# MinghanLi/UniVS

Measured on AMD Instinct MI355X. Metric: frames/sec per node, 720p T=5 clip, Swin-T 100Q; mask-logit max-abs-err, higher is better.
Workload: dtype f32; 1 GPU; BASELINE config 2: Swin-T UniVS, T=5 @ 720p (736x1280 padded), 100 queries, first clip (no prompt queries); one clip per GPU; frames_per_clip=5, queries=100, parallelism=clip-replicas x1

## Files before the change

### univs_amd/_lib.py

```python
import ctypes
import os
import re

import torch

_HERE = os.path.dirname(os.path.abspath(__file__))
LIB_PATH = os.environ.get("UNIVS_HIP_LIB") or os.path.join(_HERE, "libunivs_hip.so")

OK = 0
ERR_INVALID_ARGUMENT = -1
ERR_NOT_IMPLEMENTED = -2
ERR_LAUNCH = -3

HEADER_PATH = os.path.join(_HERE, "..", "include", "univs_hip.h")
_SCALARS = {"int": ctypes.c_int, "int32_t": ctypes.c_int, "long long": ctypes.c_longlong, "float": ctypes.c_float,
            "uint32_t": ctypes.c_uint32}
_RETURNS = {"int": ctypes.c_int, "long long": ctypes.c_longlong, "const char*": ctypes.c_char_p}
_STRUCT = r"typedef struct UnivsConfig \{(.*?)\} UnivsConfig;"


def strip_header(text):
    text = re.sub(r"/\*.*?\*/|//[^\n]*", "", text, flags=re.S)
    return re.sub(r"^[ \t]*(#.*|extern \"C\" \{|\})[ \t]*$", "", text, flags=re.M)


def parse_signatures(text):
    def ctype(words, table, name):
        t = " ".join(words).replace(" *", "*")
        if t.endswith("*") and table is _SCALARS:
            return ctypes.c_void_p
        if t not in table:
            raise TypeError(f"{name}: type {t!r} in include/univs_hip.h has no ctypes mapping")
        return table[t]

    sigs = {}
    text = re.sub(_STRUCT, "", strip_header(text), flags=re.S)
    for ret, name, params in re.findall(r"([\w \t*]+?)\b(univs_\w+)\s*\(([^)]*)\)\s*;", text):
        params = [] if params.strip() == "void" else [p.replace("*", " * ").split()[:-1] for p in params.split(",")]
        sigs[name] = (ctype(ret.replace("*", " * ").split(), _RETURNS, name), [ctype(p, _SCALARS, name) for p in params])
    return sigs


def parse_config_fields(text):
    fields = []
    for decl in re.search(_STRUCT, strip_header(text), flags=re.S).group(1).split(";")[:-1]:
        m = re.fullmatch(r"\s*int\s+(\w+)\s*(?:\[(\d+)\])?\s*", decl)
        if not m:
            raise TypeError(f"UnivsConfig: member {decl.strip()!r} in include/univs_hip.h is not an int or an int array")
        fields.append((m.group(1), ctypes.c_int * int(m.group(2)) if m.group(2) else ctypes.c_int))
    return fields


with open(HEADER_PATH) as _f:
    _HEADER = _f.read()
SIGNATURES = parse_signatures(_HEADER)
CONFIG_FIELDS = parse_config_fields(_HEADER)
EVAL_HEADER_PATH = os.path.join(_HERE, "..", "include", "univs_eval_hip.h")
with open(EVAL_HEADER_PATH) as _f:
    EVAL_SIGNATURES = parse_signatures(_f.read())

_lib = None


class UnivsHipError(RuntimeError):
    pass


def load():
    global _lib
    if _lib is not None:
        return _lib
    if not os.path.exists(LIB_PATH):
        raise UnivsHipError(
            f"{LIB_PATH} not found: the HIP extension is mandatory (no CPU fallback). "
            "Build it with `python -m univs_amd.build`.")
    lib = ctypes.CDLL(LIB_PATH)
    for name, (res, args) in (*SIGNATURES.items(), *EVAL_SIGNATURES.items()):
        fn = getattr(lib, name)
        fn.restype = res
        fn.argtypes = args
    _lib = lib
    return lib


def check(rc, what):
    if rc == OK:
        return
    msg = load().univs_last_error().decode("utf-8", "replace")
    if rc == ERR_NOT_IMPLEMENTED:
        raise NotImplementedError(f"{what}: {msg}")
    raise UnivsHipError(f"{what} failed (code {rc}): {msg}")
```

### univs_amd/build.py

```python
import os
import shutil
import subprocess
import sys

HERE = os.path.dirname(os.path.abspath(__file__))
CSRC = os.path.join(HERE, "csrc")
LIB = os.path.join(HERE, "libunivs_hip.so")
SOURCES = ["capi.hip", "msda_fwd.hip", "msda_tiled2.hip", "msda_strips.hip", "msda_heads.hip", "msda_bwd.hip", "msda_prepare.hip", "mask_decode.hip", "linear_split.hip", "linear_f16x3.hip", "gemm_f16x3_stream.hip", "gemm_f16x3_tile.hip", "mlp_f16x3.hip", "small_linear.hip", "cross_attn.hip", "window_attn.hip", "window_attn_f16.hip", "resample.hip", "semantic_extract.hip", "layer_norm.hip", "group_norm.hip", "softmax.hip", "proca_attn.hip", "prompt_sampler.hip", "transpose.hip", "mask_stats.hip", "image_post.hip", "video_post.hip", "pair_count.hip", "vss_count.hip", "davis_count.hip", "vis_overlap.hip"]
HEADERS = [os.path.join(CSRC, "common.h"), os.path.join(CSRC, "msda_common.h"), os.path.join(CSRC, "msda_geometry.h"), os.path.join(CSRC, "msda_dev.h"), os.path.join(CSRC, "msda_window_geom.h"), os.path.join(CSRC, "msda_strips_geom.h"), os.path.join(CSRC, "msda_heads_geom.h"), os.path.join(CSRC, "config.h"), os.path.join(CSRC, "window_attn.h"), os.path.join(CSRC, "f16x3.h"), os.path.join(CSRC, "gemm_plan.h"), os.path.join(CSRC, "resample_taps.h"),
           os.path.join(CSRC, "mask_post.h"), os.path.join(CSRC, "count_core.h"), os.path.join(CSRC, "launchers.h"), os.path.join(HERE, "..", "include", "univs_hip.h"),
           os.path.join(HERE, "..", "include", "univs_eval_hip.h")]


def _hipcc():
    for c in (os.environ.get("HIPCC"), shutil.which("hipcc"), "/opt/rocm/bin/hipcc"):
        if c and os.path.exists(c):
            return c
    raise RuntimeError("hipcc not found (set HIPCC or install ROCm)")


def needs_build():
    if not os.path.exists(LIB):
        return True
    t = os.path.getmtime(LIB)
    deps = [os.path.join(CSRC, s) for s in SOURCES if os.path.exists(os.path.join(CSRC, s))] + HEADERS
    return any(os.path.getmtime(d) > t for d in deps)


def _flags(defines=()):
    return ["--offload-arch=gfx950", "-O3", "-std=c++17", "-fPIC", "-fno-gpu-rdc", "-Wall", "-Wno-unused-function",
            "-I", os.path.join(HERE, "..", "include"), *[f"-D{d}" for d in defines]]


def build(force=False, verbose=True, lib=LIB, defines=(), tag=""):
    if not force and not defines and not needs_build():
        return lib
    from concurrent.futures import ThreadPoolExecutor
    objdir = os.path.join(HERE, "_obj" + tag)
    os.makedirs(objdir, exist_ok=True)
    hipcc = _hipcc()
    hdr_t = max(os.path.getmtime(h) for h in HEADERS)
    srcs = [s for s in SOURCES if os.path.exists(os.path.join(CSRC, s))]

    def compile_one(s):
        src, obj = os.path.join(CSRC, s), os.path.join(objdir, s.replace(".hip", ".o"))
        if not force and os.path.exists(obj) and os.path.getmtime(obj) > max(os.path.getmtime(src), hdr_t):
            return obj
        cmd = [hipcc, *_flags(defines), "-c", src, "-o", obj]
        if verbose:
            print("[univs_amd.build]", " ".join(cmd), file=sys.stderr, flush=True)
        subprocess.run(cmd, check=True)
        return obj

    with ThreadPoolExecutor(max_workers=min(8, os.cpu_count() or 2)) as ex:
        objs = list(ex.map(compile_one, srcs))
    cmd = [hipcc, "--offload-arch=gfx950", "-fPIC", "-shared", "-fno-gpu-rdc", *objs, "-o", lib + ".tmp"]
    if verbose:
        print("[univs_amd.build]", " ".join(cmd), file=sys.stderr, flush=True)
    subprocess.run(cmd, check=True)
    os.replace(lib + ".tmp", lib)
    return lib


ABLATIONS = {"plainsplit": ("UNIVS_SPLIT_PLAIN",), "nosplit": ("UNIVS_ABLATE_NOSPLIT",), "nomfma": ("UNIVS_ABLATE_NOMFMA",),
# ... 21 lines not shown
```

### univs_amd/csrc/capi.hip

```cpp
#include <stdarg.h>
#include <string.h>

#include <mutex>

#include "../../include/univs_eval_hip.h"
#include "common.h"
#include "config.h"
#include "launchers.h"

namespace univs {

static thread_local char g_err[512] = "";

void set_error(const char* fmt, ...) {
  va_list ap;
  va_start(ap, fmt);
  vsnprintf(g_err, sizeof(g_err), fmt, ap);
  va_end(ap);
}

static void report(const char* name, const char* fmt, va_list ap) {
  const int n = snprintf(g_err, sizeof(g_err), "%s: ", name);
  if (n >= 0 && (size_t)n < sizeof(g_err)) vsnprintf(g_err + n, sizeof(g_err) - (size_t)n, fmt, ap);
}

__attribute__((format(printf, 2, 3))) static int invalid_argument(const char* name, const char* fmt, ...) {
  va_list ap;
  va_start(ap, fmt);
  report(name, fmt, ap);
  va_end(ap);
  return UNIVS_ERR_INVALID_ARGUMENT;
}

struct Entry {
  const char* name;
  hipStream_t st;
  Entry(const char* name_, void* stream) : name(name_), st(static_cast<hipStream_t>(stream)) { clear_sticky_error(); }

  __attribute__((format(printf, 2, 3))) int invalid(const char* fmt, ...) const {
    va_list ap;
    va_start(ap, fmt);
    report(name, fmt, ap);
    va_end(ap);
    return UNIVS_ERR_INVALID_ARGUMENT;
  }
  int null_pointer() const { return invalid("NULL data pointer"); }
  __attribute__((format(printf, 3, 4))) int covered(int rc, const char* fmt, ...) const {
    if (rc != UNIVS_ERR_NOT_IMPLEMENTED) return rc;
    va_list ap;
    va_start(ap, fmt);
    report(name, fmt, ap);
    va_end(ap);
    return rc;
  }
  __attribute__((format(printf, 3, 4))) int launched(int rc, const char* fmt, ...) const {
    if (rc != 0) return rc > 0 ? UNIVS_OK : rc;
    va_list ap;
    va_start(ap, fmt);
// ... 190 lines not shown
}

int univs_small_mlp_presplit_f32(const float* x, int stages, const void* const* wp, const float* const* winv, const float* const* bias,
                                 const int* relu, const float* in_ln_weight, const float* in_ln_bias, float in_ln_eps, float* x_normed,
                                 long long M, int out_T, float* y, void* stream) {
  const Entry e("univs_small_mlp_presplit_f32", stream);
  if (M < 0 || stages < 1 || stages > 3 || out_T < 0) return e.invalid("bad arguments M=%lld stages=%d out_T=%d", M, stages, out_T);
  if (M == 0) return UNIVS_OK;
  if (!x || !y || !wp || !winv || !bias || !relu) return e.invalid("NULL pointer");
  return e.covered(small_chain_f32(x, stages, wp, winv, bias, relu, in_ln_weight, in_ln_bias, in_ln_eps, x_normed, y, M, out_T, e.st),
                   "M=%lld not covered (M <= 1 048 560, out_T | M, 16-byte aligned pointers, x_normed / bias only with a LayerNorm)", M);
}

int univs_linear_presplit_f32(const float* x, const void* wp, const float* winv, const float* bias, const float* residual,
                              long long M, int N, int K, int act, float* y, void* stream) {
  const Entry e("univs_linear_presplit_f32", stream);
  return linear_entry(e, M, N, K, act, residual, x && wp && winv && y, false, [&](int epi) {
    int rc = UNIVS_ERR_NOT_IMPLEMENTED;
    if (config().linear_ablate != 6) rc = linear_f16x3_tile_f32(x, wp, winv, bias, residual, y, M, N, K, epi, e.st);
    if (rc == UNIVS_ERR_NOT_IMPLEMENTED) rc = linear_f16x3_stream_f32(x, wp, winv, bias, residual, y, M, N, K, epi, e.st);
    return rc;
  });
}

int univs_linear_resident_presplit_f32(const float* x, const void* wp, const float* winv, const float* bias, const float* residual,
                                       long long M, int N, int K, int act, float* y, void* stream) {
  const Entry e("univs_linear_resident_presplit_f32", stream);
  return linear_entry(e, M, N, K, act, residual, x && wp && winv && y, true, [&](int epi) {
    return linear_split_f32(x, static_cast<const float*>(wp), bias, residual, y, M, N, K, epi, e.st, 0, 0, winv);
  });
}

int univs_linear_blocked_presplit_f32(const float* x, const void* wp, const float* winv, const float* bias, long long M, int N, int K,
                                      int rows_per_batch, int col_block, float* y, void* stream) {
  const Entry e("univs_linear_blocked_presplit_f32", stream);
  return linear_blocked_entry(e, M, N, K, rows_per_batch, col_block, x && wp && winv && y, [&] {
    return linear_split_f32(x, static_cast<const float*>(wp), bias, nullptr, y, M, N, K, 4, e.st, rows_per_batch, col_block,
                            winv);
  });
}

int univs_conv3x3_presplit_f32(const float* x, const void* wp, const float* winv, int T, int Cin, int Cout, int H, int W,
                               float* y, void* stream) {
  const Entry e("univs_conv3x3_presplit_f32", stream);
  return conv_entry(e, "Cin % 128, Cout % 16, >= 4096 pixels", T, Cin, Cout, H, W, x && wp && winv && y,
                    [&] { return conv3x3_f16x3_f32(x, wp, winv, y, T, Cin, Cout, H, W, e.st); });
}

int univs_conv3x3_nhwc_presplit_f32(const float* x, const void* wp, const float* winv, int T, int Cin, int Cout, int H, int W,
                                    float* y, void* stream) {
  const Entry e("univs_conv3x3_nhwc_presplit_f32", stream);
  return conv_entry(e, "Cin % 128, Cout % 16, >= 4096 pixels", T, Cin, Cout, H, W, x && wp && winv && y,
                    [&] { return conv3x3_nhwc_f16x3_f32(x, wp, winv, y, T, Cin, Cout, H, W, e.st); });
}

int univs_patch_embed4_f32(const float* x, const float* weight, const float* bias, const float* ln_weight, const float* ln_bias, float ln_eps,
                           int T, int H, int W, int E, float* out, void* stream) {
  const Entry e("univs_patch_embed4_f32", stream);
  if (T < 0 || H < 0 || W < 0 || E < 1) return e.invalid("bad dimensions T=%d H=%d W=%d E=%d", T, H, W, E);
  if (T == 0 || H == 0 || W == 0) return UNIVS_OK;
  if (!x || !weight || !out) return e.null_pointer();
  return e.covered(patch_embed4_f32(x, weight, bias, ln_weight, ln_bias, ln_eps, out, T, H, W, E, e.st),
                   "T=%d H=%d W=%d E=%d not covered (E in 96 / 128 / 192, H %% 4, W %% 4, 16-byte alignment)", T, H, W, E);
}

int univs_decoder_memory_f32(const float* x, const float* level_embed, const float* pos_yx, const float* pos_t, int T, int C, int HW,
                             float* memory, float* key, void* stream) {
  const Entry e("univs_decoder_memory_f32", stream);
  if (T < 0 || C < 0 || HW < 0) return e.invalid("bad dimensions T=%d C=%d HW=%d", T, C, HW);
  if (T == 0 || C == 0 || HW == 0) return UNIVS_OK;
  if (!x || !level_embed || !pos_yx || !pos_t || !memory || !key) return e.null_pointer();
  return e.covered(decoder_memory_f32(x, level_embed, pos_yx, pos_t, memory, key, T, C, HW, e.st),
                   "T=%d C=%d HW=%d not covered (C %% 4, HW %% 4, 16-byte alignment)", T, C, HW);
}

int univs_transpose_f32(const float* x, long long B, int R, int C, float* out, void* stream) {
  return univs_transpose_strided_f32(x, B, R, C, 0, out, stream);
}

int univs_transpose_strided_f32(const float* x, long long B, int R, int C, long long in_batch_stride, float* out, void* stream) {
  return univs_transpose_ex_f32(x, B, R, C, in_batch_stride, nullptr, out, 0, nullptr, nullptr, stream);
}

int univs_transpose_ex_f32(const float* x, long long B, int R, int C, long long in_batch_stride, const float* row_affine, float* out,
                           long long out_batch_stride, const float* addend, float* out2, void* stream) {
  const Entry e("univs_transpose_f32", stream);
  if (B < 0 || R < 0 || C < 0 || in_batch_stride < 0 || (in_batch_stride != 0 && in_batch_stride < (long long)R * C) ||
      out_batch_stride < 0 || (out_batch_stride != 0 && out_batch_stride < (long long)R * C))
    return e.invalid("bad dimensions B=%lld R=%d C=%d in_batch_stride=%lld out_batch_stride=%lld", B, R, C, in_batch_stride, out_batch_stride);
  if (B == 0 || R == 0 || C == 0) return UNIVS_OK;
  if (!x || !out || (addend != nullptr) != (out2 != nullptr)) return e.invalid("NULL data pointer (addend and out2 come together)");
  return e.covered(transpose_f32(x, out, B, R, C, in_batch_stride, out_batch_stride, row_affine, addend, out2, e.st),
                   "R=%d C=%d B=%lld not covered (R %% 4, C %% 4, strides %% 4, B <= 65535, 16-byte alignment)", R, C, B);
}

int univs_mask_decode_set_impl(int impl) {
  clear_sticky_error();
  if (impl < 0 || impl > 2) return invalid_argument(__func__, "impl=%d not in {0,1,2}", impl);
  {
    std::lock_guard<std::mutex> lock(g_cfg_mu);
    g_cfg.mask_decode_impl = impl;
  }
  return UNIVS_OK;
}

int univs_mask_decode_last_impl(void) { return mask_decode_last_impl(); }
// ... 564 lines not shown
```

### univs_amd/csrc/cross_attn.hip

```cpp
#include "common.h"
#include "launchers.h"
#include "config.h"
#include "f16x3.h"

#include <algorithm>

namespace univs {

typedef _Float16 xa_h4 __attribute__((ext_vector_type(4)));
typedef unsigned xa_u2 __attribute__((ext_vector_type(2)));

struct XaArgs {
  const float* q;
  const float* k;
  const float* v;
  const unsigned char* mask;
  const unsigned* flags;
  unsigned gen;
  float* ws;
  float* out;
  int L, S, N, H, nseg;
  int Lfull, l0;
  int ldq, ldk, ldv;
  float qscale;
};

constexpr int XA_PART = 34;
#ifndef UNIVS_XA_VS
#define UNIVS_XA_VS 36
#endif
constexpr int XA_VS = UNIVS_XA_VS;

__device__ __forceinline__ void xa_wave_scale(float mx, float& s, float& inv, int emin = -40, int emax = 128) {
#pragma unroll
  for (int off = 32; off >= 1; off >>= 1) mx = fmaxf(mx, __shfl_xor(mx, off, 64));
  int e = (int)((__builtin_bit_cast(unsigned, mx) >> 23) & 255u) - 127;
  e = max(emin, min(e, emax));
  s = __builtin_bit_cast(float, __builtin_amdgcn_readfirstlane((127 + 14 - e) << 23));
  inv = __builtin_bit_cast(float, __builtin_amdgcn_readfirstlane((127 - 14 + e) << 23));
}
__device__ __forceinline__ bool xa_out_of_range(float mx, float lo) {
  return __builtin_amdgcn_ballot_w64(!(mx < 32768.0f)) != 0 || __builtin_amdgcn_ballot_w64(mx >= lo) == 0;
}
__device__ __forceinline__ f32x4 xa_mask_init(unsigned mw, float ninf) {
  float c0, c1, c2, c3;
  asm("v_cmp_ne_u32_sdwa vcc, %4, 0 src0_sel:BYTE_0 src1_sel:DWORD\n\t"
      "v_cndmask_b32 %0, 0, %5, vcc\n\t"
      "v_cmp_ne_u32_sdwa vcc, %4, 0 src0_sel:BYTE_1 src1_sel:DWORD\n\t"
      "v_cndmask_b32 %1, 0, %5, vcc\n\t"
      "v_cmp_ne_u32_sdwa vcc, %4, 0 src0_sel:BYTE_2 src1_sel:DWORD\n\t"
      "v_cndmask_b32 %2, 0, %5, vcc\n\t"
      "v_cmp_ne_u32_sdwa vcc, %4, 0 src0_sel:BYTE_3 src1_sel:DWORD\n\t"
      "v_cndmask_b32 %3, 0, %5, vcc\n\t"
      "s_nop 1"
      : "=&v"(c0), "=&v"(c1), "=&v"(c2), "=&v"(c3)
      : "v"(mw), "v"(ninf)
      : "vcc");
  return (f32x4){c0, c1, c2, c3};
}
__device__ __forceinline__ float xa_col_max(float v) {
  const xa_u2 s1 = __builtin_amdgcn_permlane32_swap(__float_as_uint(v), __float_as_uint(v), false, false);
  const float r1 = fmaxf(__uint_as_float(s1.x), __uint_as_float(s1.y));
  const xa_u2 s2 = __builtin_amdgcn_permlane16_swap(__float_as_uint(r1), __float_as_uint(r1), false, false);
  return fmaxf(__uint_as_float(s2.x), __uint_as_float(s2.y));
}
__device__ __forceinline__ float xa_col_sum(float v) {
  const xa_u2 s1 = __builtin_amdgcn_permlane32_swap(__float_as_uint(v), __float_as_uint(v), false, false);
  const float r1 = __uint_as_float(s1.x) + __uint_as_float(s1.y);
  const xa_u2 s2 = __builtin_amdgcn_permlane16_swap(__float_as_uint(r1), __float_as_uint(r1), false, false);
  return __uint_as_float(s2.x) + __uint_as_float(s2.y);
}

template <int NQB>
__global__ __launch_bounds__(64, 2) void xattn_partial(const XaArgs a) {
  constexpr int HD = 32;
  __shared__ __attribute__((aligned(16))) _Float16 vt[2 * HD * XA_VS];
  __shared__ __attribute__((aligned(16))) f16x8 qlds[2 * NQB * 64];
  const int lane = threadIdx.x;
  const int j = lane & 15, g = lane >> 4;
  const int seg = blockIdx.x, nh = blockIdx.y, chunk = blockIdx.z;
// ... 252 lines not shown
        }
      lsum[qb] += part;
      f16x8 ph, pm;
      l3_split8<true>(pv, ph, pm);
#pragma unroll
      for (int hf = 0; hf < 2; ++hf) {
        f32x4 o = oacc[qb][hf];
        if (v_scaled) {
          asm volatile("; rare");
          o *= sv_fwd;
        }
        o = __builtin_amdgcn_mfma_f32_16x16x32_f16(pm, vh[hf], o, 0, 0, 0);
        o = __builtin_amdgcn_mfma_f32_16x16x32_f16(ph, vm[hf], o, 0, 0, 0);
        o = __builtin_amdgcn_mfma_f32_16x16x32_f16(ph, vh[hf], o, 0, 0, 0);
        if (v_scaled) {
          asm volatile("; rare");
          o *= sv_inv;
        }
        oacc[qb][hf] = o;
      }
    }
  }

  float* wsb = a.ws + (((long long)chunk * gridDim.y + nh) * a.nseg + seg) * (16 * NQB) * XA_PART;
#pragma unroll
  for (int qb = 0; qb < NQB; ++qb) {
    const float ltot = xa_col_sum(lsum[qb]);
#pragma unroll
    for (int r = 0; r < 4; ++r) {
      float* p = wsb + (long long)(16 * qb + 4 * g + r) * XA_PART;
      p[j] = oacc[qb][0][r];
      p[16 + j] = oacc[qb][1][r];
    }
    if (g == 0) {
      float* p = wsb + (long long)(16 * qb + j) * XA_PART;
      p[32] = mref[qb];
      p[33] = ltot;
    }
  }
}

__global__ __launch_bounds__(256) void xattn_merge(const float* __restrict__ ws, float* __restrict__ out, int L, int Lp, int N, int H, int nseg) {
  const long long idx = (long long)blockIdx.x * 256 + threadIdx.x;
  const long long total = (long long)N * H * L * 32;
  if (idx >= total) return;
  const int c = (int)(idx & 31);
  const long long t = idx >> 5;
  const int q = (int)(t % L);
  const int nh = (int)(t / L);
  const int n = nh / H, h = nh - n * H;
  const int chunk = q / Lp, ql = q - chunk * Lp;
  const float* base = ws + ((((long long)chunk * N * H + nh) * nseg) * Lp + ql) * XA_PART;
  const long long pstride = (long long)Lp * XA_PART;
  float M = -INFINITY;
#pragma unroll 8
  for (int p = 0; p < nseg; ++p) M = fmaxf(M, base[p * pstride + 32]);
  float acc = 0.f, l = 0.f;
#pragma unroll 8
  for (int p = 0; p < nseg; ++p) {
    const float f = __builtin_amdgcn_exp2f(base[p * pstride + 32] - M);
    acc = fmaf(base[p * pstride + c], f, acc);
    l = fmaf(base[p * pstride + 33], f, l);
  }
  out[((long long)q * N + n) * (H * 32) + h * 32 + c] = acc / l;
}

constexpr int XA_MAX_NQB = 7;
struct XaPlan {
  int nseg, nqb;
};
static XaPlan xa_plan(int L, int S, int N, int H) {
  const int nit = (S + 31) / 32, blocks = (L + 15) / 16;
  const int cfg = std::max(0, config().xattn_segments);
  const int forced = cfg & 0xffff, forced_nqb = std::min((cfg >> 16) & 0xf, XA_MAX_NQB);
  const double KV = 2.2, PROLOGUE = 0.5, MERGE = 0.2 / 4480.0;
  const long long simds = 4LL * cu_count();
  XaPlan best{1, 1};
  double best_t = 1e300;
  for (int nqb = 1; nqb <= std::min(blocks, XA_MAX_NQB); ++nqb) {
    if (forced_nqb > 0 && nqb != std::min(forced_nqb, blocks)) continue;
    const long long groups = (long long)N * H * ((blocks + nqb - 1) / nqb);
    int nseg = (int)std::max<long long>(1, std::min<long long>(std::min(nit, nit / 2), 2 * simds / groups));
    if (nseg >= 8) nseg -= nseg % 8;
    if (forced > 0) nseg = std::min(forced, nit);
    const int iters = (nit + nseg - 1) / nseg;
    const double per_simd = (double)groups * nseg / (double)simds;
    const double t = (iters * (KV + nqb) + PROLOGUE * nqb) * std::max(1.0, per_simd / 2) + MERGE * nseg * (double)(groups * 16 * nqb);
    if (t < best_t) {
      best_t = t;
      best = XaPlan{nseg, nqb};
    }
  }
  return best;
}

size_t cross_attention_workspace_floats(int L, int S, int N, int H) {
  const XaPlan p = xa_plan(L, S, N, H);
  const int nchunks = (L + 16 * p.nqb - 1) / (16 * p.nqb);
  return (size_t)nchunks * N * H * p.nseg * (16 * p.nqb) * XA_PART;
}

int cross_attention_f32(const float* q, const float* k, const float* v, const unsigned char* mask, const unsigned* row_flags,
                        unsigned generation, int L, int S, int N, int H, int hd, int ldq, int ldk, int ldv, float scale, float* ws,
                        float* out, hipStream_t st) {
  if (L <= 0 || N <= 0 || H <= 0) return UNIVS_OK;
  auto mis = [](const void* p) { return (reinterpret_cast<uintptr_t>(p) & 15) != 0; };
  if (hd != 32 || S < 32 || (mask && ((row_flags && S % 4 != 0) || (reinterpret_cast<uintptr_t>(mask) & 3))) || mis(q) || mis(k) || mis(v) || mis(out) ||
      mis(ws) || (long long)N * H > 65535)
    return UNIVS_ERR_NOT_IMPLEMENTED;
  const XaPlan plan = xa_plan(L, S, N, H);
  const int nseg = plan.nseg, nqb = plan.nqb;
  const int E = H * 32;
  ldq = ldq > 0 ? ldq : E; ldk = ldk > 0 ? ldk : E; ldv = ldv > 0 ? ldv : E;
  if (ldq < E || ldk < E || ldv < E || ldq % 4 || ldk % 4 || ldv % 4) return UNIVS_ERR_NOT_IMPLEMENTED;
  const int nchunks = (L + 16 * nqb - 1) / (16 * nqb);
  if (nchunks > 65535) return UNIVS_ERR_NOT_IMPLEMENTED;
  XaArgs a{};
  a.q = q; a.k = k; a.v = v;
  a.mask = mask;
  a.flags = mask ? row_flags : nullptr;
  a.gen = generation;
  a.ws = ws; a.out = out;
  a.L = L; a.S = S; a.N = N; a.H = H; a.nseg = nseg;
  a.Lfull = L; a.l0 = 0;
  a.ldq = ldq; a.ldk = ldk; a.ldv = ldv;
  a.qscale = scale * 1.4426950408889634f;
  dim3 grid((unsigned)nseg, (unsigned)(N * H), (unsigned)nchunks);
  switch (nqb) {
    case 1: hipLaunchKernelGGL(xattn_partial<1>, grid, dim3(64), 0, st, a); break;
    case 2: hipLaunchKernelGGL(xattn_partial<2>, grid, dim3(64), 0, st, a); break;
    case 3: hipLaunchKernelGGL(xattn_partial<3>, grid, dim3(64), 0, st, a); break;
    case 4: hipLaunchKernelGGL(xattn_partial<4>, grid, dim3(64), 0, st, a); break;
    case 5: hipLaunchKernelGGL(xattn_partial<5>, grid, dim3(64), 0, st, a); break;
    case 6: hipLaunchKernelGGL(xattn_partial<6>, grid, dim3(64), 0, st, a); break;
    default: hipLaunchKernelGGL(xattn_partial<7>, grid, dim3(64), 0, st, a); break;
  }
  int rc = check_launch("xattn_partial");
  if (rc != UNIVS_OK) return rc;
  const long long total = (long long)N * H * L * 32;
  hipLaunchKernelGGL(xattn_merge, dim3((unsigned)((total + 255) / 256)), dim3(256), 0, st, ws, out, L, 16 * nqb, N, H, nseg);
  return check_launch("xattn_merge");
}

}
```

### univs_amd/csrc/gemm_f16x3_stream.hip

```cpp
#include "common.h"
#include "config.h"
#include "f16x3.h"
#include "gemm_plan.h"
#include "launchers.h"

#include <algorithm>
#include <cstdlib>

namespace univs {

#ifdef UNIVS_TRACE_GEMM
UNIVS_GT_DECL(g_gs_trace);
#endif
enum { GS_EPI_NONE = EPI_NONE, GS_EPI_RELU = EPI_RELU, GS_EPI_GELU = EPI_GELU, GS_EPI_RESIDUAL = EPI_RESIDUAL };

__global__ __launch_bounds__(256) void presplit_f16x3_kernel(const float* __restrict__ W, int N, int K, int conv_cin, int kperm,
                                                             u32x4* __restrict__ Wp, float* __restrict__ winv) {
  __shared__ unsigned smax;
  const int r = blockIdx.x;
  if (threadIdx.x == 0) smax = 0u;
  __syncthreads();
  const float* src = W + (size_t)r * K;
  auto elem = [&](int k) __attribute__((always_inline)) -> float {
    if (conv_cin == 0) return src[k];
    const int tap = k / conv_cin, ci = k - tap * conv_cin;
    return src[ci * 9 + tap];
  };
  unsigned mx = 0u;
  for (int k = threadIdx.x; k < K; k += blockDim.x) mx = max(mx, __builtin_bit_cast(unsigned, fabsf(elem(k))));
  atomicMax(&smax, mx);
  __syncthreads();
  float s, inv;
  l3_scale(smax, 14, s, inv);
  if (threadIdx.x == 0) winv[r] = inv;
  for (int kc = threadIdx.x; kc < (K >> 3); kc += blockDim.x) {
    f32x4 v0, v1;
#pragma unroll
    for (int e = 0; e < 4; ++e) {
      const int k0 = kperm ? (kc >> 2) * 32 + 4 * (kc & 3) + e : kc * 8 + e;
      v0[e] = elem(k0);
      v1[e] = elem(kperm ? k0 + 16 : k0 + 4);
    }
    f16x8 h, m;
    l3_split8(v0, v1, s, h, m);
    Wp[(size_t)(kc * 2) * N + r] = __builtin_bit_cast(u32x4, h);
    Wp[(size_t)(kc * 2 + 1) * N + r] = __builtin_bit_cast(u32x4, m);
  }
}

int presplit_f16x3(const float* w, int N, int K, int conv_cin, int kperm, void* wp, float* winv, hipStream_t st) {
  if (N <= 0) return UNIVS_OK;
  hipLaunchKernelGGL(presplit_f16x3_kernel, dim3(N), dim3(256), 0, st, w, N, K, conv_cin, kperm, reinterpret_cast<u32x4*>(wp), winv);
  return check_launch("presplit_f16x3");
}

struct GsArgs {
  const float* X;
  const u32x4* Wp;
  const float* winv;
  const float* bias;
  const float* Res;
  float* Y;
  int M, N, K, rows_per_pass, epi;
  int Cin, Cout, H, Wd, HW;
  int tap0;
  int remap;
};

template <int RB, int RING, int XMODE>
__global__ __launch_bounds__(GS_THREADS, 512 / GS_THREADS) void gemm_f16x3_stream(const GsArgs a) {
  extern __shared__ __attribute__((aligned(16))) u32x4 Wst[];
  [[maybe_unused]] const int gts = UNIVS_GT_SLOT();
  UNIVS_GT(g_gs_trace, gts, 0);
  UNIVS_GT_REAL(g_gs_trace, gts, 62);
  constexpr int Rp = 16 * RB;
  constexpr int SLAB = RING * 4 * 2 * Rp;
  unsigned bx = blockIdx.x, by = blockIdx.y;
  if (a.remap && gridDim.y > 1) {
    const unsigned lw = xcd_remap(blockIdx.x + gridDim.x * blockIdx.y, gridDim.x * gridDim.y);
    bx = lw / gridDim.y;
    by = lw - bx * gridDim.y;
  }
  const int n0 = by * a.rows_per_pass;
  const int R = min(a.rows_per_pass, a.N - n0);
  const int tid = threadIdx.x, lane = tid & 63;
  const int wave = __builtin_amdgcn_readfirstlane(tid >> 6);
  const int M = a.M, N = a.N, K = a.K, epi = a.epi;
  const int KS = K >> 5, KG = KS / RING;
  const int j = lane & 15, g = lane >> 4;
  float* bias_lds = reinterpret_cast<float*>(Wst + 2 * SLAB);
  float* winv_lds = bias_lds + Rp;
  constexpr int NWV = GS_THREADS / 64;

  const int WT = (M + GS_TILE_M - 1) / GS_TILE_M;
  const int wg0 = (int)((long long)WT * bx / gridDim.x), wg1 = (int)((long long)WT * (bx + 1) / gridDim.x);
  const int rounds = (wg1 - wg0 + NWV - 1) / NWV;
  if (rounds == 0) return;

  for (int r = tid; r < Rp; r += GS_THREADS) {
    bias_lds[r] = (a.bias && r < R) ? a.bias[n0 + r] : 0.f;
    winv_lds[r] = r < R ? a.winv[n0 + r] : 0.f;
  }

  constexpr int UNITS = RING * 8 * Rp;
  constexpr int UPT = (UNITS + GS_THREADS - 1) / GS_THREADS;
  constexpr int UPS = (UPT + RING - 1) / RING;
  u32x4 wreg[UPS];
  auto w_fetch = [&](int q, int u) __attribute__((always_inline)) {
#pragma unroll
    for (int v = 0; v < UPS; ++v) {
      const int i = tid + GS_THREADS * (u * UPS + v);
      const int run = i / Rp, rr = i - run * Rp;
      wreg[v] = (u32x4){0u, 0u, 0u, 0u};
      if (u * UPS + v < UPT && i < UNITS && rr < R) wreg[v] = a.Wp[(size_t)(q * RING * 8 + run) * N + n0 + rr];
    }
  };
  auto w_commit = [&](int buf, int u) __attribute__((always_inline)) {
#pragma unroll
    for (int v = 0; v < UPS; ++v) {
      const int i = tid + GS_THREADS * (u * UPS + v);
      if (u * UPS + v < UPT && i < UNITS) Wst[buf * SLAB + i] = wreg[v];
    }
  };
#pragma unroll
  for (int u = 0; u < RING; ++u) {
    w_fetch(0, u);
    w_commit(0, u);
  }

  const long long xbytes = XMODE == 0 ? (long long)M * K * 4 : (long long)(M / a.HW) * a.Cin * a.HW * 4;
  const __amdgpu_buffer_rsrc_t xrs = __builtin_amdgcn_make_buffer_rsrc(const_cast<float*>(a.X), 0, (int)xbytes, 0x00020000);
  const long long ybytes = XMODE == 0 ? (long long)M * N * 4 : (long long)(M / a.HW) * a.Cout * a.HW * 4;
  const __amdgpu_buffer_rsrc_t yrs = __builtin_amdgcn_make_buffer_rsrc(a.Y, 0, (int)ybytes, 0x00020000);
  const __amdgpu_buffer_rsrc_t rrs =
      __builtin_amdgcn_make_buffer_rsrc(const_cast<float*>(epi == GS_EPI_RESIDUAL ? a.Res : a.X), 0, (int)ybytes, 0x00020000);

  struct TileRows {
    unsigned vo[2];
    int py[2], px[2];
  };
  auto tile_rows = [&](int tt, TileRows& t) __attribute__((always_inline)) {
#pragma unroll
    for (int c = 0; c < 2; ++c) {
      const int m = min(tt * GS_TILE_M + 16 * c + j, M - 1);
      if (XMODE == 0) {
        t.vo[c] = ((unsigned)m * (unsigned)K + (unsigned)(8 * g)) * 4u;
        t.py[c] = t.px[c] = 0;
      } else if (XMODE == 2) {
        const int f = m / a.HW, rem = m - f * a.HW;
        t.py[c] = rem / a.Wd;
        t.px[c] = rem - t.py[c] * a.Wd;
        t.vo[c] = ((unsigned)m * (unsigned)a.Cin + (unsigned)(8 * g)) * 4u;
      } else {
        const int f = m / a.HW, rem = m - f * a.HW;
        t.py[c] = rem / a.Wd;
        t.px[c] = rem - t.py[c] * a.Wd;
        t.vo[c] = (unsigned)((f * a.Cin + 8 * g) * a.HW + rem) * 4u;
      }
    }
  };
  f32x4 raw[RING][2][2];
  const int kspt = XMODE != 0 ? a.Cin >> 5 : 1;
  auto load_x = [&](f32x4 (&buf)[2][2], const TileRows& t, int ks) __attribute__((always_inline)) {
    if (XMODE == 0) {
#pragma unroll
      for (int c = 0; c < 2; ++c) {
        buf[c][0] = __builtin_bit_cast(f32x4, __builtin_amdgcn_raw_buffer_load_b128(xrs, t.vo[c], ks * 128, 0));
        buf[c][1] = __builtin_bit_cast(f32x4, __builtin_amdgcn_raw_buffer_load_b128(xrs, t.vo[c] + 16u, ks * 128, 0));
      }
    } else if (XMODE == 2) {
      const int tap_ = ks / kspt, cb = (ks - tap_ * kspt) * 32;
      const int tap = tap_ + a.tap0;
      const int dy = tap / 3 - 1, dx = tap - (tap / 3) * 3 - 1;
#pragma unroll
      for (int c = 0; c < 2; ++c) {
        const bool inb = (unsigned)(t.py[c] + dy) < (unsigned)a.H && (unsigned)(t.px[c] + dx) < (unsigned)a.Wd;
        const unsigned vo = inb ? t.vo[c] + (unsigned)((dy * a.Wd + dx) * a.Cin * 4) : 0xFFFFFFE0u;
        buf[c][0] = __builtin_bit_cast(f32x4, __builtin_amdgcn_raw_buffer_load_b128(xrs, vo, cb * 4, 0));
        buf[c][1] = __builtin_bit_cast(f32x4, __builtin_amdgcn_raw_buffer_load_b128(xrs, vo + 16u, cb * 4, 0));
      }
    } else {
      const int tap_ = ks / kspt, cb = (ks - tap_ * kspt) * 32;
      const int tap = tap_ + a.tap0;
      const int dy = tap / 3 - 1, dx = tap - (tap / 3) * 3 - 1;
#pragma unroll
      for (int c = 0; c < 2; ++c) {
        const bool inb = (unsigned)(t.py[c] + dy) < (unsigned)a.H && (unsigned)(t.px[c] + dx) < (unsigned)a.Wd;
        const unsigned vo = inb ? t.vo[c] + (unsigned)((dy * a.Wd + dx) * 4) : 0xFFFFFFF0u;
#pragma unroll
        for (int e = 0; e < 8; ++e)
          buf[c][e >> 2][e & 3] = __builtin_bit_cast(float, __builtin_amdgcn_raw_buffer_load_b32(xrs, vo, (cb + e) * a.HW * 4, 0));
      }
    }
  };

  f32x4 acc[RB][2];
  int eset[2];
  float sx[2], sx_inv[2];
  constexpr int NB = RB > 6 ? 4 : 2;
  constexpr int BSZ = (RB + NB - 1) / NB;
  u32x4 afr[2][BSZ][2];
  const unsigned a_lane = (unsigned)((g * 2 * Rp + j) * 16);
  const unsigned a_kstep = (unsigned)(8 * Rp * 16);
  const unsigned a_part = (unsigned)(Rp * 16);
  auto read_batch = [&](u32x4 (&d)[BSZ][2], unsigned base, auto bc) __attribute__((always_inline)) {
    constexpr int b = decltype(bc)::value;
    l3_static_for<0, BSZ>([&](auto qc) __attribute__((always_inline)) {
      constexpr int q = decltype(qc)::value;
      constexpr int rb = b * BSZ + q < RB ? b * BSZ + q : RB - 1;
      u32x4& dh = d[q][0];
      u32x4& dm = d[q][1];
      const unsigned aa = base;
      asm volatile("ds_read_b128 %0, %2 offset:%3\n\tds_read_b128 %1, %2 offset:%4"
                   : "=&v"(dh), "=&v"(dm)
                   : "v"(aa), "n"(rb * 256), "n"(rb * 256 + Rp * 16)
                   : "memory");
    });
  };
  auto wait_batch = [&](u32x4 (&d)[BSZ][2]) __attribute__((always_inline)) {
    if constexpr (BSZ == 1)
      asm volatile("s_waitcnt lgkmcnt(0)" : "+v"(d[0][0]), "+v"(d[0][1]) : : "memory");
    else if constexpr (BSZ == 2)
      asm volatile("s_waitcnt lgkmcnt(0)" : "+v"(d[0][0]), "+v"(d[0][1]), "+v"(d[1][0]), "+v"(d[1][1]) : : "memory");
    else
      asm volatile("s_waitcnt lgkmcnt(0)"
                   : "+v"(d[0][0]), "+v"(d[0][1]), "+v"(d[1][0]), "+v"(d[1][1]), "+v"(d[2][0]), "+v"(d[2][1]) : : "memory");
  };

  TileRows t_cur, t_next;
  tile_rows(wg0 + wave, t_cur);
  tile_rows(wg0 + min(1, rounds - 1) * NWV + wave, t_next);
#pragma unroll
  for (int u = 0; u < RING; ++u) load_x(raw[u], t_cur, u);

  UNIVS_GT(g_gs_trace, gts, 2);
  UNIVS_GT_VAL(g_gs_trace, gts, 63, rounds);
  int gq = 0;
#pragma unroll 1
  for (int rd = 0; rd < rounds; ++rd) {
    const int tt = wg0 + rd * NWV + wave;
    const bool tile_ok = tt < wg1;
#pragma unroll
    for (int rb = 0; rb < RB; ++rb) acc[rb][0] = acc[rb][1] = (f32x4){0.f, 0.f, 0.f, 0.f};
    eset[0] = eset[1] = -1000;
    sx[0] = sx[1] = sx_inv[0] = sx_inv[1] = 1.0f;
#pragma unroll 1
    for (int q = 0; q < KG; ++q, ++gq) {
      __syncthreads();
      const int bufc = gq & 1, qn = (q + 1 == KG) ? 0 : q + 1;
      const bool last_group = q + 1 == KG;
      const unsigned a_buf = a_lane + (unsigned)(bufc * SLAB * 16);
      read_batch(afr[0], a_buf, std::integral_constant<int, 0>{});
#pragma unroll
      for (int u = 0; u < RING; ++u) {
        if (u > 0) w_commit(bufc ^ 1, u - 1);
        bool need = false;
        int enew[2];
#pragma unroll
        for (int c = 0; c < 2; ++c) {
          const unsigned mk = l3_row_max(l3_absmax8(raw[u][c][0], raw[u][c][1]));
          enew[c] = max(-100, min((int)((mk >> 23) & 255u) - 127, 128));
          need = need || (enew[c] > eset[c] + 2);
        }
        if (__builtin_amdgcn_ballot_w64(need) != 0) {
#pragma unroll
          for (int c = 0; c < 2; ++c) {
            const bool mine = enew[c] > eset[c] + 2;
            const int en = mine ? enew[c] : eset[c];
            const float ratio = __builtin_bit_cast(float, (unsigned)(127 + max(eset[c] - en, -126)) << 23);
#pragma unroll
            for (int rb = 0; rb < RB; ++rb) acc[rb][c] *= ratio;
            eset[c] = en;
            sx[c] = __builtin_bit_cast(float, (unsigned)(127 + 12 - en) << 23);
            sx_inv[c] = __builtin_bit_cast(float, (unsigned)(127 - 12 + en) << 23);
          }
        }
        float s0 = sx[0], s1 = sx[1];
        asm volatile("" : "+v"(s0), "+v"(s1) : : "memory");
        f16x8 bh[2], bm[2];
        l3_split8(raw[u][0][0], raw[u][0][1], s0, bh[0], bm[0]);
        l3_split8(raw[u][1][0], raw[u][1][1], s1, bh[1], bm[1]);
        __builtin_amdgcn_sched_barrier(0);
        w_fetch(qn, u);
        if (last_group) load_x(raw[u], t_next, u);
        else load_x(raw[u], t_cur, q * RING + u + RING);
        __builtin_amdgcn_sched_barrier(0);
        l3_static_for<0, NB>([&](auto bc) __attribute__((always_inline)) {
          constexpr int b = decltype(bc)::value;
          wait_batch(afr[b & 1]);
          if constexpr (b + 1 < NB) read_batch(afr[(b + 1) & 1], a_buf + (unsigned)u * a_kstep, std::integral_constant<int, b + 1>{});
          else if (u + 1 < RING) read_batch(afr[0], a_buf + (unsigned)(u + 1) * a_kstep, std::integral_constant<int, 0>{});
          __builtin_amdgcn_sched_barrier(0);
#pragma unroll
          for (int qq = 0; qq < BSZ; ++qq) {
            const int rb = b * BSZ + qq;
            if (rb < RB) {
              const f16x8 ah = __builtin_bit_cast(f16x8, afr[b & 1][qq][0]);
              const f16x8 am = __builtin_bit_cast(f16x8, afr[b & 1][qq][1]);
              acc[rb][0] = __builtin_amdgcn_mfma_f32_16x16x32_f16(am, bh[0], acc[rb][0], 0, 0, 0);
              acc[rb][1] = __builtin_amdgcn_mfma_f32_16x16x32_f16(am, bh[1], acc[rb][1], 0, 0, 0);
              acc[rb][0] = __builtin_amdgcn_mfma_f32_16x16x32_f16(ah, bm[0], acc[rb][0], 0, 0, 0);
              acc[rb][1] = __builtin_amdgcn_mfma_f32_16x16x32_f16(ah, bm[1], acc[rb][1], 0, 0, 0);
              acc[rb][0] = __builtin_amdgcn_mfma_f32_16x16x32_f16(ah, bh[0], acc[rb][0], 0, 0, 0);
              acc[rb][1] = __builtin_amdgcn_mfma_f32_16x16x32_f16(ah, bh[1], acc[rb][1], 0, 0, 0);
            }
          }
          __builtin_amdgcn_sched_barrier(0);
        });
// ... 11 lines not shown
        rem = min(m, M - 1) - fr * a.HW;
      }
      constexpr int RBAT = RB > 4 ? (RB + 1) / 2 : RB;
      [[maybe_unused]] f32x4 resv[RBAT];
      auto load_res = [&](int rb0) __attribute__((always_inline)) {
        if (XMODE == 0 && epi == GS_EPI_RESIDUAL) {
#pragma unroll
          for (int q = 0; q < RBAT; ++q) {
            const int f = min(rb0 + q, RB - 1) * 16 + 4 * g;
            const unsigned off = ((unsigned)m * (unsigned)N + (unsigned)(n0 + f)) * 4u;
            resv[q] = __builtin_bit_cast(f32x4, __builtin_amdgcn_raw_buffer_load_b128(rrs, (row_ok && f < R) ? off : 0xFFFFFFF0u, 0, 0));
          }
        } else {
#pragma unroll
          for (int q = 0; q < RBAT; ++q) resv[q] = (f32x4){0.f, 0.f, 0.f, 0.f};
        }
      };
#pragma unroll
      for (int rb = 0; rb < RB; ++rb) {
        if (rb % RBAT == 0) load_res(rb);
        const int f = rb * 16 + 4 * g;
        const f32x4 wi = *reinterpret_cast<const f32x4*>(winv_lds + f);
        const f32x4 bi = *reinterpret_cast<const f32x4*>(bias_lds + f);
        f32x4 v = (acc[rb][c] * sx_inv[c]) * wi + bi;
        if (XMODE == 0) {
          const unsigned off = ((unsigned)m * (unsigned)N + (unsigned)(n0 + f)) * 4u;
          const unsigned offc = (row_ok && f < R) ? off : 0xFFFFFFF0u;
          if (epi == GS_EPI_RELU) v = __builtin_elementwise_maximum(v, (f32x4){0.f, 0.f, 0.f, 0.f})   ;
          if (epi == GS_EPI_GELU) {
#pragma unroll
            for (int e = 0; e < 4; ++e) v[e] = l3_gelu(v[e]);
          }
          if (epi == GS_EPI_RESIDUAL) v += resv[rb % RBAT];
          __builtin_amdgcn_raw_buffer_store_b128(__builtin_bit_cast(u32x4, v), yrs, offc, 0, 0);
        } else {
          const unsigned off0 = (row_ok && f < R) ? (unsigned)((fr * a.Cout + n0 + f) * a.HW + rem) * 4u
                                                  : 0xFFFFFFF0u - 3u * (unsigned)a.HW * 4u;
          float vx = v.x, vy = v.y, vz = v.z, vw = v.w;
          asm volatile("" : "+v"(vx), "+v"(vy), "+v"(vz), "+v"(vw));
          __builtin_amdgcn_raw_buffer_store_b32(__builtin_bit_cast(unsigned, vx), yrs, off0, 0, 0);
          __builtin_amdgcn_raw_buffer_store_b32(__builtin_bit_cast(unsigned, vy), yrs, off0 + (unsigned)a.HW * 4u, 0, 0);
          __builtin_amdgcn_raw_buffer_store_b32(__builtin_bit_cast(unsigned, vz), yrs, off0 + 2u * (unsigned)a.HW * 4u, 0, 0);
          __builtin_amdgcn_raw_buffer_store_b32(__builtin_bit_cast(unsigned, vw), yrs, off0 + 3u * (unsigned)a.HW * 4u, 0, 0);
        }
      }
    }
    UNIVS_GT(g_gs_trace, gts, 4 + 2 * rd);
    t_cur = t_next;
    tile_rows(wg0 + min(rd + 2, rounds - 1) * NWV + wave, t_next);
  }
  UNIVS_GT_REAL(g_gs_trace, gts, 61);
}

template <int XMODE>
static int gs_launch(const GsArgs& a0, hipStream_t st) {
  GsArgs a = a0;
  const StreamPlan p = plan_stream(XMODE, a.M, a.N, a.K, cu_count(), config());
  a.rows_per_pass = p.rows_per_pass;
  a.remap = p.remap;
  const int RB = p.RB, ring = p.ring;
  const size_t lds = p.lds;
  dim3 grid(p.gx, p.passes), block(GS_THREADS);
#define UNIVS_GS(rb, rg)                                                                                          \
  do {                                                                                                            \
    (void)hipFuncSetAttribute(reinterpret_cast<const void*>(&gemm_f16x3_stream<rb, rg, XMODE>),                   \
                              hipFuncAttributeMaxDynamicSharedMemorySize, (int)lds);                              \
    hipLaunchKernelGGL((gemm_f16x3_stream<rb, rg, XMODE>), grid, block, lds, st, a);                              \
  } while (0)
#define UNIVS_GS_RB(rb)                    \
  case rb:                                 \
    if (ring == 4) { UNIVS_GS(rb, 4); }    \
    else { UNIVS_GS(rb, 3); }              \
    break
  switch (RB) {
    UNIVS_GS_RB(1);
    UNIVS_GS_RB(2);
    UNIVS_GS_RB(3);
    UNIVS_GS_RB(4);
    UNIVS_GS_RB(5);
    UNIVS_GS_RB(6);
    UNIVS_GS_RB(7);
    default: UNIVS_GS_RB(8);
  }
#undef UNIVS_GS_RB
#undef UNIVS_GS
  return check_launch("gemm_f16x3_stream");
}

int linear_f16x3_stream_f32(const float* x, const void* wp, const float* winv, const float* bias, const float* residual, float* y,
                            long long M, int N, int K, int epi, hipStream_t st) {
  if (M <= 0 || N <= 0) return UNIVS_OK;
  if (!epi_consistent(epi, EPI_RESIDUAL, residual != nullptr) || !stream_linear_covered(M, N, K) ||
      !aligned16(x, wp, y, residual, bias, winv))
    return UNIVS_ERR_NOT_IMPLEMENTED;
  GsArgs a{};
  a.X = x; a.Wp = reinterpret_cast<const u32x4*>(wp); a.winv = winv; a.bias = bias; a.Res = residual; a.Y = y;
  a.M = (int)M; a.N = N; a.K = K; a.epi = epi;
  return gs_launch<0>(a, st);
}

template <int XMODE>
static int gs_conv(const float* x, const void* wp, const float* winv, const float* bias, float* y, int T, int Cin, int Cout, int H, int W,
                   int taps, hipStream_t st) {
  if (T <= 0 || Cout <= 0 || H <= 0 || W <= 0) return UNIVS_OK;
  const long long M = (long long)T * H * W;
  if (!stream_conv_covered(M, Cin, Cout, taps) || !aligned16(x, wp, y, winv, bias)) return UNIVS_ERR_NOT_IMPLEMENTED;
  GsArgs a{};
  a.X = x; a.Wp = reinterpret_cast<const u32x4*>(wp); a.winv = winv; a.bias = bias; a.Res = nullptr; a.Y = y;
  a.M = (int)M; a.N = Cout; a.K = taps * Cin; a.epi = GS_EPI_NONE;
  a.Cin = Cin; a.Cout = Cout; a.H = H; a.Wd = W; a.HW = H * W;
  a.tap0 = taps == 9 ? 0 : 4;
  return gs_launch<XMODE>(a, st);
}

int conv3x3_f16x3_f32(const float* x, const void* wp, const float* winv, float* y, int T, int Cin, int Cout, int H, int W,
                      hipStream_t st) {
  return gs_conv<1>(x, wp, winv, nullptr, y, T, Cin, Cout, H, W, 9, st);
}

int conv3x3_nhwc_f16x3_f32(const float* x, const void* wp, const float* winv, float* y, int T, int Cin, int Cout, int H, int W,
                           hipStream_t st) {
  return gs_conv<2>(x, wp, winv, nullptr, y, T, Cin, Cout, H, W, 9, st);
}

int conv1x1_f16x3_f32(const float* x, const void* wp, const float* winv, const float* bias, float* y, int T, int Cin, int Cout, int H,
                      int W, hipStream_t st) {
  return gs_conv<1>(x, wp, winv, bias, y, T, Cin, Cout, H, W, 1, st);
}

}

#ifdef UNIVS_TRACE_GEMM
extern "C" int univs_debug_gemm_trace_stream(unsigned long long* out, int clear) {
  if (clear) {
    static unsigned long long zeros[UNIVS_GT_SLOTS * UNIVS_GT_STAMPS] = {};
    return (int)hipMemcpyToSymbol(HIP_SYMBOL(univs::g_gs_trace), zeros, sizeof(zeros));
  }
  (void)hipDeviceSynchronize();
  return (int)hipMemcpyFromSymbol(out, HIP_SYMBOL(univs::g_gs_trace), sizeof(unsigned long long) * UNIVS_GT_SLOTS * UNIVS_GT_STAMPS);
}
#endif
```

### univs_amd/csrc/gemm_plan.h

```cpp
#pragma once
#include <stddef.h>
#include <stdint.h>

#include <algorithm>

#include "../../include/univs_hip.h"

namespace univs {

constexpr int LS_THREADS = 512;
constexpr int LS_TILE_M = 32;
constexpr int LS_MAX_RB = 7;
constexpr int L3_THREADS = 512;
constexpr int L3_TILE_M = 32;
constexpr int L3_MAX_RB = 8;
constexpr int L3_WPT = 24;
#ifndef UNIVS_GS_THREADS
#define UNIVS_GS_THREADS 512
#endif
constexpr int GS_THREADS = UNIVS_GS_THREADS;
constexpr int GS_TILE_M = 32;
constexpr int GT_THREADS = 512;
enum { EPI_NONE = 0, EPI_RELU = 1, EPI_GELU = 2, EPI_RESIDUAL = 3, EPI_BLOCKED = 4 };

// ... 36 lines not shown
  return (M + LS_TILE_M - 1) / LS_TILE_M >= 64;
}
inline bool resident_six_products(const UnivsConfig& cfg, bool presplit) { return cfg.linear_terms == 6 && !presplit; }
struct ResidentPlan {
  bool covered;
  int RB, ksc, ring;
  unsigned gx, passes;
  size_t lds;
  int rows_per_pass;
};
constexpr long long RESIDENT_LDS_CAP = 160 * 1024 - 2048;
inline ResidentPlan plan_bf16x6_resident(long long M, int N, int K, int epi, int n_cu) {
  ResidentPlan p{};
  int r_cap = (int)std::min<long long>(RESIDENT_LDS_CAP / ((long long)K * 6), 16 * LS_MAX_RB);
  r_cap -= r_cap % 4;
  if (r_cap < 16) return p;
  const PassPlan pp = plan_passes(N, r_cap, 4);
  const long long WT = (M + LS_TILE_M - 1) / LS_TILE_M;
  p.covered = true;
  p.RB = pp.RB;
  p.ksc = (epi == EPI_BLOCKED || K == 256) ? 8 : 0;
  p.ring = p.ksc ? 4 : k_ring(K);
  p.gx = (unsigned)plan_row_ranges(n_cu, pp.passes, WT, LS_THREADS / 64, 2, 0);
  p.passes = (unsigned)pp.passes;
  p.lds = (size_t)K * pp.rows * 6 + 4 * (size_t)pp.rows + 16 * 48 + 16;
  p.rows_per_pass = pp.rows;
  return p;
}
inline ResidentPlan plan_f16x3_resident(long long M, int N, int K, bool presplit, int n_cu, const UnivsConfig& cfg) {
  ResidentPlan p{};
  int r_cap = (int)std::min<long long>(RESIDENT_LDS_CAP / ((long long)K * 4 + 12), 16 * L3_MAX_RB);
  r_cap -= r_cap % 16;
  if (cfg.linear_rows_per_pass >= 16) r_cap = std::min(r_cap, cfg.linear_rows_per_pass - cfg.linear_rows_per_pass % 16);
  if (r_cap < 16) return p;
  const PassPlan pp = plan_passes(N, r_cap, 4);
  if (presplit && ((K >> 3) * 2 + (L3_THREADS / pp.rows) - 1) / (L3_THREADS / pp.rows) > L3_WPT) return p;
  const long long WT = (M + L3_TILE_M - 1) / L3_TILE_M;
  p.covered = true;
  p.RB = pp.RB;
  p.ring = k_ring(K);
  p.gx = (unsigned)plan_row_ranges(n_cu, pp.passes, WT, L3_THREADS / 64, 2, cfg.linear_grid_x);
  p.passes = (unsigned)pp.passes;
  p.lds = (size_t)K * (16 * pp.RB) * 4 + 12 * (size_t)pp.rows + 256 + 16;
  p.rows_per_pass = pp.rows;
  return p;
}

inline bool stream_linear_covered(long long M, int N, int K) {
  return k_ring(K) != 0 && K >= 96 && N % 4 == 0 && M >= 2048 && fits_int32(M, N) && fits_int32(M, K);
}
inline bool stream_conv_covered(long long M, int Cin, int Cout, int taps) {
  return (taps == 9 ? Cin % 128 == 0 : k_ring(Cin) != 0) && Cout % 16 == 0 && M >= 4096 && fits_int32(M, std::max(Cin, Cout));
}
struct StreamPlan {
  int RB, ring;
  unsigned gx, passes;
  size_t lds;
  int rows_per_pass, remap;
};
inline StreamPlan plan_stream(int xmode, long long M, int N, int K, int n_cu, const UnivsConfig& cfg) {
  StreamPlan p{};
  const bool narrow = xmode == 0 && N <= 768 && K >= N && M <= 32768;
  const int r_cap = cfg.linear_rows_per_pass >= 16 ? std::min(128, cfg.linear_rows_per_pass - cfg.linear_rows_per_pass % 16)
                                                   : (narrow ? 64 : 128);
  const PassPlan pp = plan_passes(N, r_cap, xmode != 0 ? 16 : 4);
  const long long WT = (M + GS_TILE_M - 1) / GS_TILE_M;
  long long gx = plan_row_ranges(n_cu, pp.passes, WT, GS_THREADS / 64, 1, cfg.linear_grid_x);
  p.RB = pp.RB;
  p.ring = k_ring(K);
  p.lds = (size_t)2 * p.ring * 8 * (16 * pp.RB) * 16 + 8 * (size_t)(16 * pp.RB);
  if (GS_THREADS < 512 && cfg.linear_grid_x <= 0 && p.lds * (512 / GS_THREADS) <= 156 * 1024)
    gx = std::min<long long>(gx * (512 / GS_THREADS), std::max<long long>(1, WT / (GS_THREADS / 64)));
  p.gx = (unsigned)gx;
  p.passes = (unsigned)pp.passes;
  p.rows_per_pass = pp.rows;
  p.remap = cfg.linear_ablate == 5 ? 0 : 1;
  return p;
}

struct TilePlan {
  bool covered;
  int ct, rb, nslot, occ;
  unsigned grid;
  size_t lds;
  int tf, nf;
};
constexpr bool tile_occ2(int ct, int rb) { return (ct == 3 && rb <= 3) || (ct == 4 && rb == 2); }
inline TilePlan plan_tile(long long M, int N, int K, int n_cu, const UnivsConfig& cfg) {
  TilePlan p{};
  if (K % 64 != 0 || K < 384 || N % 4 != 0 || N < 128 || M < 2048 || !fits_int32(M, N) || !fits_int32(M, K) || !fits_int32(K, N)) return p;
  int nslot = K % 128 == 0 ? 4 : K % 96 == 0 ? 3 : 2;
  if (cfg.linear_ablate >= 7 && cfg.linear_ablate <= 9 && K % (32 * (cfg.linear_ablate - 5)) == 0) nslot = cfg.linear_ablate - 5;
  int best_occ = 1;
  double best_t = 1e300;
  for (int ct = 3; ct <= 5; ++ct)
    for (int rb = 2; rb <= 4; ++rb) {
      if (cfg.linear_grid_x >= 3 && cfg.linear_grid_x <= 5 && ct != cfg.linear_grid_x) continue;
      if (cfg.linear_rows_per_pass >= 128 && rb != std::min(4, cfg.linear_rows_per_pass / 64)) continue;
      const int nf = (N + 64 * rb - 1) / (64 * rb);
      int tf = (N + nf - 1) / nf;
      tf = (tf + 3) & ~3;
      if ((tf + 63) / 64 != rb) continue;
      const int occ = tile_occ2(ct, rb) ? 2 : 1;
      const long long wgs = ((M + 32 * ct - 1) / (32 * ct)) * nf;
      const double ks = K / 32;
      const double mfma = 2.0 * ct * rb * 3 * 16;
// ... 21 lines not shown
```

### univs_amd/csrc/launchers.h

```cpp
#pragma once
#include "common.h"

namespace univs {

int msda_forward_generic_f32(const float* value, const LevelTable& lv, const float* loc,
                             const float* attn, int N, int S, int M, int D, int L, int Lq, int P,
                             float* out, hipStream_t st);
int msda_forward_generic_f64(const double* value, const LevelTable& lv, const double* loc,
                             const double* attn, int N, int S, int M, int D, int L, int Lq, int P,
                             double* out, hipStream_t st);

int msda_forward_tiled2_f32(const float* value, const LevelTable& lv, const float* loc, const float* attn, int N,
                            int S, int M, int D, int L, int Lq, int P, float* out, hipStream_t st);

int msda_forward_strips_f32(const float* vhm, const LevelTable& lv, const float* qhm, const float* ref,
                            long long ref_batch_stride, int N, int S, int M, int D, int L, int Lq, int P, float* out,
                            hipStream_t st);

int msda_forward_heads_f32(const float* vhm, const LevelTable& lv, const float* qhm, const float* ref,
                           long long ref_batch_stride, int N, int S, int M, int D, int L, int Lq, int P, float* out,
                           hipStream_t st);

int msda_backward_f32(const float* value, const LevelTable& lv, const float* loc, const float* attn,
                      const float* grad_out, int N, int S, int M, int D, int L, int Lq, int P, float* grad_value,
                      float* grad_loc, float* grad_attn, hipStream_t st);

int msda_prepare_f32(const float* qp, int row_stride, int n_off, const float* ref, long long ref_batch_stride,
                     const LevelTable& lv, int N, int Lq, int M, int L, int P, float* loc, float* attn, hipStream_t st);

int mask_decode_f32(const float* mask_embed, const float* mask_features, int T, int Q, int C,
                    long long HW, float* out, hipStream_t st);
int mask_decode_last_impl();
int mask_decode_attn_f32(const float* mask_embed, const float* feat_lowres, int T, int Q, int C,
                         long long hw, uint8_t* attn_mask, unsigned* row_any_ws, unsigned generation, hipStream_t st);
int attn_mask_rows_reset(uint8_t* attn_mask, const unsigned* row_flags, unsigned generation, long long rows, long long hw, hipStream_t st);

int linear_split_f32(const float* x, const float* w, const float* bias, const float* residual, float* y, long long M, int N,
                     int K, int epi, hipStream_t st, int blk_rows = 0, int blk_cols = 0, const float* winv = nullptr);

int linear_f16x3_f32(const float* x, const float* w, const float* bias, const float* residual, float* y, long long M, int N,
                     int K, int epi, hipStream_t st, int blk_rows, int blk_cols, const float* winv, int n_cu);

int conv3x3_nhwc_f16x3_f32(const float* x, const void* wp, const float* winv, float* y, int T, int Cin, int Cout, int H, int W,
                           hipStream_t st);
int presplit_f16x3(const float* w, int N, int K, int conv_cin, int kperm, void* wp, float* winv, hipStream_t st);
int linear_f16x3_stream_f32(const float* x, const void* wp, const float* winv, const float* bias, const float* residual, float* y,
                            long long M, int N, int K, int epi, hipStream_t st);
int conv3x3_f16x3_f32(const float* x, const void* wp, const float* winv, float* y, int T, int Cin, int Cout, int H, int W,
                      hipStream_t st);
int conv1x1_f16x3_f32(const float* x, const void* wp, const float* winv, const float* bias, float* y, int T, int Cin, int Cout, int H,
                      int W, hipStream_t st);

int linear_f16x3_tile_f32(const float* x, const void* wp, const float* winv, const float* bias, const float* residual, float* y,
                          long long M, int N, int K, int epi, hipStream_t st);

int mlp_f16x3_f32(const float* x, const void* w1p, const float* w1inv, const float* b1, const void* w2p, const float* w2inv,
                  const float* b2, const float* residual, const float* ln_w, const float* ln_b, float ln_eps, const float* pln_w,
                  const float* pln_b, float pln_eps, const float* post_add, long long post_add_rows, float* y2, float* y, long long M,
                  int C, int Hd, int act, int flags, hipStream_t st);

int small_chain_f32(const float* x, int stages, const void* const* wp, const float* const* winv, const float* const* bias, const int* relu,
                    const float* in_g, const float* in_b, float in_eps, float* xn, float* y, long long M, int out_T, hipStream_t st);
int small_linear_f32(const float* x, const float* xadd, const void* wp, const float* winv, const float* bias, int n_w, int f_off,
                     const float* residual, const float* ln_g, const float* ln_b, float ln_eps, float* y, long long M, int N, int K,
                     int relu, int add_features, int out_T, hipStream_t st);

int cross_attention_f32(const float* q, const float* k, const float* v, const unsigned char* mask, const unsigned* row_flags,
                        unsigned generation, int L, int S, int N, int H, int hd, int ldq, int ldk, int ldv, float scale, float* ws,
                        float* out, hipStream_t st);
size_t cross_attention_workspace_floats(int L, int S, int N, int H);

int window_attention_image_f32(const float* qkv, const float* qkv_bias, const float* bias, const float* shift_mask,
                               int B, int H, int W, int ws, int shift, int nH, int hd, float scale, float* out,
                               hipStream_t st);
int window_attention_f32(const float* qkv, const float* bias, const float* shift_mask, int B_, int nW,
                         int Ntok, int nH, int hd, float scale, float* out, hipStream_t st);

int window_attention_image_f16mma(const float* qkv, const float* qkv_bias, const float* bias, const float* shift_mask, int B,
                                  int H, int W, int ws, int shift, int nH, int hd, float scale, int terms, float* out,
                                  hipStream_t st);

int bilinear_resample_f32(const float* in, const float* addend, float* out, long long planes, int Hin, int Win,
                          int Hout, int Wout, hipStream_t st);
int upsample2x_add_f32(const float* in, const float* addend, const float* affine, float* out, long long planes, int Hin, int Win,
                       hipStream_t st);
int normalize_pad_f32(const float* in, float* out, long long T, int C, int H, int W, int Hp, int Wp, const float* mean, const float* stdv,
                      hipStream_t st);
int bilinear_pyramid3_f32(const float* in, float* out2, float* out4, float* out8, long long planes, int H, int W, hipStream_t st);

int bilinear_crop_nearest_f32(const float* in, float* out, int C, int h, int w, int Hp, int Wp, int Hi, int Wi, int hc, int wc, int t_first,
                              int t_step, int K, hipStream_t st);

int layer_norm_f32(const float* x, const float* res, const float* gamma, const float* beta, long long rows, int C,
                   float eps, float* sum_out, float* out, const float* addend, float* out2, long long addend_rows, hipStream_t st);
int patch_merge_norm_f32(const float* x, const float* gamma, const float* beta, int B, int H, int W, int C, float eps, float* out,
                         hipStream_t st);

int group_norm_affine_f32(const float* x, const float* gamma, const float* beta, int N, int C, long long HW, int groups, float eps,
                          float* ws, long long ws_floats, float* affine, hipStream_t st);
int group_norm_f32(const float* x, const float* gamma, const float* beta, int N, int C, long long HW, int groups,
                   float eps, int relu, float* ws, long long ws_floats, float* out, hipStream_t st);

int masked_softmax_f32(float* scores, const unsigned char* mask, int N, int h, int L, int S, hipStream_t st);

int proca_attention_f32(const float* qkv0, const float* kd, const float* vd, int Qp, int L, int T, int h, int hd, float scale,
                        float* out, hipStream_t st);

int prompt_prefix_f32(const float* masks, const float* boxes, int Fk, int n, int h, int w, int scale, float feat_thresh,
                      float* feat_masks, unsigned* stats, uint8_t* sel, int* rowcnt, uint8_t* fmb, int* counts, uint8_t* valid,
                      uint8_t* visible, hipStream_t st);
int prompt_draw(const uint8_t* sel, const int* rowcnt, const uint8_t* fmb, const int* counts, const float* u, const float* keys,
                const long long* tab, int Fk, int n, int h, int w, int HW, int R, long long* point_idx, long long* dense_idx,
                uint8_t* empty, float* point_coords, hipStream_t st);
int prompt_point_pe_f32(const float* xy, const float* z, const float* dim_t, const float* dim_tz, float scale, int Fk, int n, int F,
                        float* out, hipStream_t st);
int token_mean_f32(const float* x, const float* add, int n, int L, int T, int C, float* out, hipStream_t st);
int prompt_tokens_f32(const float* feats, const long long* fs, const float* pos, const long long* ps, const float* qfeat,
                      const float* qpe, const long long* dense_idx, const uint8_t* empty, const uint8_t* valid, const float* boxes,
                      const long long* kf, int Fk, int n, int R, int T, int C, int h_img, int w_img, float* fd, float* pd, uint8_t* attn,
                      hipStream_t st);

int transpose_f32(const float* in, float* out, long long B, int R, int C, long long in_bstride, long long out_bstride,
// ... 44 lines not shown
```

### univs_amd/csrc/small_linear.hip

```cpp
#include "common.h"
#include "f16x3.h"
#include "launchers.h"

#include <algorithm>
#include <cstdlib>

namespace univs {

constexpr int SL_WAVES = 8;
constexpr int SL_AHEAD = 4;
constexpr int SL_KMAX = 256;

struct SlArgs {
  const float* X;
  const float* Xadd;
  const u32x4* Wp;
  const float* winv;
  const float* bias;
  const float* Res;
  const float* ln_g;
  const float* ln_b;
  float ln_eps;
  float* Y;
  int M, N, K, Nw, f_off, relu;
  int out_T;
  int add_features;
};

typedef unsigned sl_u2 __attribute__((ext_vector_type(2)));
__device__ __forceinline__ float sl_row_sum(float v) {
  const sl_u2 s1 = __builtin_amdgcn_permlane32_swap(__float_as_uint(v), __float_as_uint(v), false, false);
  const float r1 = __uint_as_float(s1.x) + __uint_as_float(s1.y);
  const sl_u2 s2 = __builtin_amdgcn_permlane16_swap(__float_as_uint(r1), __float_as_uint(r1), false, false);
  return __uint_as_float(s2.x) + __uint_as_float(s2.y);
}

__global__ __launch_bounds__(64 * SL_WAVES, 3) void small_linear_kernel(const SlArgs a) {
  extern __shared__ __attribute__((aligned(16))) u32x4 xs[];
  __shared__ float red[2][SL_WAVES][16];
  __shared__ unsigned rmax[2][16];
  __shared__ float rinv[2][16];
  const int tid = threadIdx.x, lane = tid & 63;
  const int wave = __builtin_amdgcn_readfirstlane(tid >> 6);
  const int j = lane & 15, g = lane >> 4;
  const int M = a.M, N = a.N, K = a.K, KS = K >> 5;
  const int row0 = blockIdx.x * 16;
  const int fbase = blockIdx.y * (32 * SL_WAVES);
  const int f0 = fbase + wave * 32;
  const bool with_ln = a.ln_g != nullptr;
  const bool f_ok1 = f0 + 16 < N;
  const int fend = min(fbase + 32 * SL_WAVES, N);
  const bool need_add = a.Xadd != nullptr && (a.add_features == 0 || fbase < a.add_features);
  const bool need_plain = a.Xadd == nullptr || (a.add_features != 0 && fend > a.add_features);
  const int my_tile = (a.Xadd != nullptr && (a.add_features == 0 || f0 < a.add_features)) ? 0 : 1;
  const int tile_units = 2 * KS * 64;

  const u32x4* wl = a.Wp + (size_t)(g * 2) * a.Nw + a.f_off + min(f0, N - 16) + j;
  const size_t kstep_units = (size_t)8 * a.Nw;
  u32x4 afr[SL_AHEAD][2][2];
  auto load_a = [&](int ks, u32x4 (&d)[2][2]) __attribute__((always_inline)) {
    const u32x4* p = wl + (size_t)ks * kstep_units;
    d[0][0] = p[0];
    d[0][1] = p[a.Nw];
    d[1][0] = f_ok1 ? p[16] : p[0];
    d[1][1] = f_ok1 ? p[a.Nw + 16] : p[a.Nw];
  };
#pragma unroll
  for (int u = 0; u < SL_AHEAD; ++u)
    if (u < KS) load_a(u, afr[u]);

  if (tid < 32) (&rmax[0][0])[tid] = 0u;
  __syncthreads();
  constexpr int SLOTS = (SL_KMAX / 32) * 64 / (64 * SL_WAVES);
  f32x4 xv[SLOTS][2], xw[SLOTS][2];
#pragma unroll
  for (int i = 0; i < SLOTS; ++i) {
    const int s_ = tid + 64 * SL_WAVES * i;
    if (s_ < KS * 64) {
      const int ks = s_ >> 6, l_ = s_ & 63, j_ = l_ & 15, g_ = l_ >> 4;
      const long long off = (long long)min(row0 + j_, M - 1) * K + 32 * ks + 8 * g_;
      xv[i][0] = *reinterpret_cast<const f32x4*>(a.X + off);
      xv[i][1] = *reinterpret_cast<const f32x4*>(a.X + off + 4);
      if (need_add) {
        xw[i][0] = xv[i][0] + *reinterpret_cast<const f32x4*>(a.Xadd + off);
        xw[i][1] = xv[i][1] + *reinterpret_cast<const f32x4*>(a.Xadd + off + 4);
        atomicMax(&rmax[0][j_], l3_absmax8(xw[i][0], xw[i][1]));
      }
      if (need_plain) atomicMax(&rmax[1][j_], l3_absmax8(xv[i][0], xv[i][1]));
    }
  }
  __syncthreads();
#pragma unroll
  for (int i = 0; i < SLOTS; ++i) {
    const int s_ = tid + 64 * SL_WAVES * i;
    if (s_ < KS * 64) {
      const int j_ = s_ & 15;
      float sc, inv;
      f16x8 h8, m8;
      if (need_add) {
        l3_scale(rmax[0][j_], 14, sc, inv);
        l3_split8(xw[i][0], xw[i][1], sc, h8, m8);
        xs[s_] = __builtin_bit_cast(u32x4, h8);
        xs[KS * 64 + s_] = __builtin_bit_cast(u32x4, m8);
        if (s_ < 16) rinv[0][s_] = inv;
      }
      if (need_plain) {
        l3_scale(rmax[1][j_], 14, sc, inv);
        l3_split8(xv[i][0], xv[i][1], sc, h8, m8);
        xs[tile_units + s_] = __builtin_bit_cast(u32x4, h8);
        xs[tile_units + KS * 64 + s_] = __builtin_bit_cast(u32x4, m8);
        if (s_ < 16) rinv[1][s_] = inv;
      }
    }
  }
  __syncthreads();
  if (f0 >= N && !with_ln) return;
  const float sx_inv = rinv[my_tile][j];
  const int m = min(row0 + j, M - 1);
  const int row = row0 + j;
  const bool row_ok = row < M;
  f32x4 e_wi[2], e_bi[2], e_res[2];
#pragma unroll
  for (int q = 0; q < 2; ++q) {
    const int f = f0 + 16 * q + 4 * g;
    const bool ok = f < N;
    const int fw = a.f_off + (ok ? f : 0);
    e_wi[q] = *reinterpret_cast<const f32x4*>(a.winv + fw);
    e_bi[q] = a.bias ? *reinterpret_cast<const f32x4*>(a.bias + fw) : (f32x4){0.f, 0.f, 0.f, 0.f};
    e_res[q] = (a.Res && ok) ? *reinterpret_cast<const f32x4*>(a.Res + (long long)m * N + f) : (f32x4){0.f, 0.f, 0.f, 0.f};
  }
  const u32x4* xt = xs + my_tile * tile_units + lane;

  f32x4 acc[2] = {(f32x4){0.f, 0.f, 0.f, 0.f}, (f32x4){0.f, 0.f, 0.f, 0.f}};
#pragma unroll 1
  for (int kb = 0; kb < KS; kb += SL_AHEAD) {
// ... 34 lines not shown
    const float ws = sl_row_sum(sm);
    if (g == 0) red[0][wave][j] = ws;
    __syncthreads();
    float tot = 0.f;
#pragma unroll
    for (int w = 0; w < SL_WAVES; ++w) tot += red[0][w][j];
    const float mean = tot * inv_n;
    float sq = 0.f;
#pragma unroll
    for (int q = 0; q < 2; ++q) {
      v[q] -= mean;
#pragma unroll
      for (int e = 0; e < 4; ++e) sq = fmaf(v[q][e], v[q][e], sq);
    }
    const float wq = sl_row_sum(sq);
    if (g == 0) red[1][wave][j] = wq;
    __syncthreads();
    float tq = 0.f;
#pragma unroll
    for (int w = 0; w < SL_WAVES; ++w) tq += red[1][w][j];
    const float rstd = 1.0f / sqrtf(tq * inv_n + a.ln_eps);
#pragma unroll
    for (int q = 0; q < 2; ++q) {
      const int f = f0 + 16 * q + 4 * g;
      const f32x4 gm = *reinterpret_cast<const f32x4*>(a.ln_g + f);
      f32x4 y = (v[q] * rstd) * gm;
      if (a.ln_b) y += *reinterpret_cast<const f32x4*>(a.ln_b + f);
      v[q] = y;
    }
  }
  const int orow = a.out_T > 0 ? (row % a.out_T) * (M / a.out_T) + row / a.out_T : row;
#pragma unroll
  for (int q = 0; q < 2; ++q) {
    const int f = f0 + 16 * q + 4 * g;
    if (row_ok && f < N) *reinterpret_cast<f32x4*>(a.Y + (long long)orow * N + f) = v[q];
  }
}

int small_linear_f32(const float* x, const float* xadd, const void* wp, const float* winv, const float* bias, int n_w, int f_off,
                     const float* residual, const float* ln_g, const float* ln_b, float ln_eps, float* y, long long M, int N, int K,
                     int relu, int add_features, int out_T, hipStream_t st) {
  if (M <= 0 || N <= 0) return UNIVS_OK;
  auto mis = [](const void* p) { return (reinterpret_cast<uintptr_t>(p) & 15) != 0; };
  if (K < 32 || K % 32 != 0 || K > SL_KMAX || N % 16 != 0 || n_w % 4 != 0 || f_off % 4 != 0 || f_off < 0 || f_off + N > n_w || M > 16LL * 65535 ||
      (ln_g && N != 32 * SL_WAVES) || (ln_b && !ln_g) || add_features < 0 || add_features % 32 != 0 || out_T < 0 || (out_T > 0 && (M % out_T != 0 || residual || ln_g)) || mis(x) || mis(xadd) || mis(wp) || mis(winv) || mis(bias) || mis(residual) ||
      mis(ln_g) || mis(ln_b) || mis(y) || M * (long long)std::max(N, K) * 4 >= 0x7FFFFFFFLL)
    return UNIVS_ERR_NOT_IMPLEMENTED;
  SlArgs a{};
  a.X = x; a.Xadd = xadd; a.Wp = reinterpret_cast<const u32x4*>(wp); a.winv = winv; a.bias = bias; a.Res = residual;
  a.ln_g = ln_g; a.ln_b = ln_b; a.ln_eps = ln_eps; a.Y = y;
  a.M = (int)M; a.N = N; a.K = K; a.Nw = n_w; a.f_off = f_off; a.relu = relu ? 1 : 0; a.add_features = add_features; a.out_T = out_T;
  dim3 grid((unsigned)((M + 15) / 16), (unsigned)((N + 32 * SL_WAVES - 1) / (32 * SL_WAVES)));
  const size_t lds = (size_t)2 * 2 * (K / 32) * 64 * 16;
  hipLaunchKernelGGL(small_linear_kernel, grid, dim3(64 * SL_WAVES), lds, st, a);
  return check_launch("small_linear_f32");
}

struct SlChainArgs {
  const float* X;
  const u32x4* Wp[3];
  const float* winv[3];
  const float* bias[3];
  int relu[3];
  int stages;
  const float* in_g;
  const float* in_b;
  float in_eps;
  float* Xn;
  float* Y;
  int M, out_T;
};

__global__ __launch_bounds__(64 * SL_WAVES, 3) void small_chain_kernel(const SlChainArgs a) {
  constexpr int K = 256, N = 256, KS = K >> 5;
  __shared__ __attribute__((aligned(16))) u32x4 xs[2][2 * KS * 64];
  __shared__ unsigned rmax[3][16];
  __shared__ float rstat[2][SL_WAVES][16];
  const int tid = threadIdx.x, lane = tid & 63;
  const int wave = __builtin_amdgcn_readfirstlane(tid >> 6);
  const int j = lane & 15, g = lane >> 4;
  const int M = a.M;
  const int row0 = blockIdx.x * 16;
  const int f0 = wave * 32;

  u32x4 afr[SL_AHEAD][2][2];
  auto load_a = [&](const u32x4* wl, int ks, u32x4 (&d)[2][2]) __attribute__((always_inline)) {
    const u32x4* p = wl + (size_t)ks * (8 * N);
    d[0][0] = p[0];
    d[0][1] = p[N];
    d[1][0] = p[16];
    d[1][1] = p[N + 16];
  };
  const size_t wl_off = (size_t)(g * 2) * N + f0 + j;
#pragma unroll
  for (int u = 0; u < SL_AHEAD; ++u) load_a(a.Wp[0] + wl_off, u, afr[u]);

  if (tid < 48) (&rmax[0][0])[tid] = 0u;
  __syncthreads();
  {
    const int s_ = tid;
    const int ks = s_ >> 6, l_ = s_ & 63, j_ = l_ & 15, g_ = l_ >> 4;
    const int mrow = min(row0 + j_, M - 1);
    const long long off = (long long)mrow * K + 32 * ks + 8 * g_;
    f32x4 x0 = *reinterpret_cast<const f32x4*>(a.X + off), x1 = *reinterpret_cast<const f32x4*>(a.X + off + 4);
    if (a.in_g) {
      const float s4 = sl_row_sum(((x0[0] + x0[1]) + (x0[2] + x0[3])) + ((x1[0] + x1[1]) + (x1[2] + x1[3])));
      if (g_ == 0) rstat[0][ks][j_] = s4;
      __syncthreads();
// ... 132 lines not shown
```

### univs_amd/inference/video_entity.py

```python
import math
from typing import Tuple

import numpy as np
import torch
import torch.nn.functional as F
from torch import nn

from ..registry import configurable
from ..utils.memory import retry_if_oom
from ..layers import to_device_async
from ..utils.comm import batched_mask_iou, calculate_mask_quality_scores, convert_mask_to_box, count_true, video_box_iou
from .comm import check_consistency_with_prev_frames, match_from_learnable_embds
from scipy.optimize import linear_sum_assignment

COMBINED_DATASETS_CATEGORY_INFO = {
    "imagenet": (1000, 0), "lvis": (1203, 1000), "burst": (1203, 1000), "ytvis21": (40, 2203), "ovis": (25, 2243),
    "bdd_track": (8, 2268), "objects365": (365, 2276), "coco_panoptic": (133, 2641), "coco": (80, 2641),
    "ade20k": (150, 2774), "vipseg": (124, 2924), "vspw": (124, 2924), "viposeg": (124, 2924), "ytvis19": (40, 3048),
    "entityseg_instance": (206, 3088), "entityseg_panoptic": (644, 3294),
}
ENTITY_SUBTASK_DATASET = {
    "entity_vss_entityseg": "entityseg_panoptic",
    "entity_vps_entityseg": "entityseg_panoptic",
    "entity_vss_vipseg": "vipseg",
    "entity_vps_vipseg": "vipseg",
    "entity_vis_entityseg": "entityseg_instance",
    "entity_vis_coco": "coco",
}


class ImageList:

    def __init__(self, tensor, image_sizes):
        self.tensor, self.image_sizes = tensor, image_sizes

    @staticmethod
    def from_tensors(tensors, size_divisibility=0):
        sizes = [tuple(t.shape[-2:]) for t in tensors]
        H, W = max(s[0] for s in sizes), max(s[1] for s in sizes)
        if size_divisibility > 1:
            d = size_divisibility
            H, W = (H + d - 1) // d * d, (W + d - 1) // d * d
        out = tensors[0].new_zeros((len(tensors),) + tuple(tensors[0].shape[:-2]) + (H, W))
        for i, t in enumerate(tensors):
            out[i, ..., : t.shape[-2], : t.shape[-1]] = t
        return ImageList(out, sizes)


def normalized_image_list(frames, pixel_mean, pixel_std, size_divisibility):
    if (len(frames) > 0 and frames[0].is_cuda and frames[0].dtype == torch.float32 and frames[0].dim() == 3
            and all(f.shape == frames[0].shape for f in frames) and not torch.is_grad_enabled()):
        from .. import ops
# ... 73 lines not shown
        import torch.distributed as dist
        if t is None:
            t = torch.empty(shape, dtype=dtype, device=self.device)
        t = t.contiguous()
        if t.numel():
            dist.broadcast(t, src=self.shard.global_rank(self.team[0]), group=self.shard.group)
            if self.shard.rank != self.team[0]:
                self.shard.bytes["result:broadcast"] += t.numel() * t.element_size()
        return t

    def _index(self, idx):
        if isinstance(idx, torch.Tensor) and idx.device == self.device:
            return idx
        return to_device_async(torch.as_tensor(idx, dtype=torch.long).cpu(), self.device)

    def stats(self):
        full = None
        if self.cs is not None:
            st = _plane_stats(self.local).to(torch.int32)
            before = self.shard.bytes["all_gather"]
            full = self.cs.all_gather_frames(st, dim=1)
            self._account("all_gather", before)
        return self._to_outside(full, (self.n_rows, self.T, 8), torch.int32)

    def rows(self, idx):
        n = len(idx)
        if n == 0:
            return torch.zeros((0, self.T) + self.hw, device=self.device)
        full = None
        if self.cs is not None:
            before = self.shard.bytes["all_gather"]
            full = self.cs.all_gather_frames(self.local.index_select(0, self._index(idx)), dim=1)
            self._account("all_gather", before)
        return self._to_outside(full, (n, self.T) + self.hw, torch.float32)

    def iou_max(self, idx, known):
        n = len(idx)
        v = None
        if self.cs is not None:
            pos = torch.as_tensor(self.cs.local_positions, device=known.device)
            m = self.local.index_select(0, self._index(idx)).transpose(0, 1).gt(0.0)
            v = batched_mask_iou(m, known.index_select(0, pos)).amax(dim=(0, 2))
            before = self.shard.bytes["all_reduce"]
            v = self.cs.all_reduce_max(v)
            self._account("all_reduce", before)
        return self._to_outside(v, (n,), torch.float32)


def window_features_on_owner(model, x, frames, shard):
    mine = [f for f in frames if f % shard.world == shard.rank]
    if not mine:
        return {}, None
    feats = model.backbone(x[mine] if mine != list(range(mine[0], mine[0] + len(mine))) else x[mine[0]:mine[0] + len(mine)])
    mf, bfe, _enc, ms = model.sem_seg_head.pixel_decoder.forward_features(feats)
    return {f: k for k, f in enumerate(mine)}, (mf, bfe, list(ms))


POOL_KEYS = ("prompt_pe", "prompt_feats", "prompt_attn_masks")


def _sampler_encoder(model):
    try:
        return model.sem_seg_head.predictor.visual_prompt_sampler.visual_prompt_encoder
    except AttributeError:
        return None


def sharded_clip_forward(model, targets, first, n_clip, rows, pd, shard, device=None, lazy_masks=False):
    from ..distributed import ClipShard, cyclic_owners
    predictor = model.sem_seg_head.predictor
    if getattr(predictor, "semantic_extraction_enable", False):
        raise NotImplementedError("frame-sharded clip loop: MODEL.UniVS.TEST.SEMANTIC_EXTRACTION.ENABLE is not supported")
    owners = cyclic_owners(first, n_clip, shard.world)
    team = sorted(set(owners))
    whole = len(team) == shard.world
    group = shard.group if whole else shard.subgroup(team)
    tv = targets[0]
    out = None
    if shard.rank in team:
        cs = ClipShard([team.index(o) for o in owners], group=group, always_collective=shard.always_collective, counter=shard.bytes)
        k = [rows[first + p] for p in cs.local_positions]
        sel = (lambda t: t[k[0]:k[0] + len(k)]) if k == list(range(k[0], k[0] + len(k))) else (lambda t: t[k])
        mf, bfe, ms = pd
        predictor.frame_shard = cs
        try:
            out = predictor([sel(lv) for lv in ms], sel(mf), sel(bfe) if bfe is not None else None, None, targets)
        finally:
            predictor.frame_shard = None
        before = shard.bytes["all_gather"]
        if not lazy_masks:
            out["pred_masks"] = cs.all_gather_frames(out["pred_masks"], dim=2)
        out["pred_embds"] = cs.all_gather_frames(out["pred_embds"], dim=2)
        shard.bytes["result:all_gather"] += shard.bytes["all_gather"] - before
        shard.bytes["all_gather"] = before
        if lazy_masks:
            pm = out["pred_masks"]
            lazy = ClipMaskRows(shard, team, cs, pm[0].float().contiguous(), pm.shape[1], n_clip, pm.shape[-2:], pm.device)
    if whole:
        return (out, lazy) if lazy_masks else out
    if device is None:
        device = pd[0].device if pd is not None else torch.device("cpu")
    enc = _sampler_encoder(model)
    src = team[0]
    state = {}
    if shard.rank == src:
        state = {f"out:{k_}": v for k_, v in out.items() if isinstance(v, torch.Tensor) and not (lazy_masks and k_ == "pred_masks")}
        if lazy_masks:
# ... 155 lines not shown
        return self.dataset_category_info.get(dataset_name)

    def set_frame_shard(self, shard):
        self.frame_shard = shard

    def inference_video(self, model, batched_inputs, images, targets, merge_results=True, on_clip=None):
        x = images.tensor
        tv = targets[0]
        sub_task = tv["sub_task"]
        if not any(t in sub_task for t in ("vis", "vss", "vps")):
            raise ValueError(f"Not support to eval the sub-task {sub_task!r} yet")
        n_total = len(x)
        video_len = int(batched_inputs[0]["video_len"])
        interim_size = tuple(x.shape[-2:])
        image_size = tuple(images.image_sizes[0])
        out_size = (batched_inputs[0].get("height", image_size[0]), batched_inputs[0].get("width", image_size[1]))
        T = self.num_frames
        stride = min(T if "vss" in sub_task else self.clip_stride, T)

        results = []
        is_last = False
        win_start = win_end = 0
        feats_window = None
        shard = check_loop_shard(getattr(self, "frame_shard", None), T)
        lazy_ok = shard is not None and "vis" in sub_task and self.use_quasi_track and not getattr(self, "replicate_clip_masks", False)
        lazy = None
        begin_video(model, x.device, shard)
        win_rows, win_pd = {}, None
        for i in range(0, n_total, stride):
            if is_last and i + T > n_total:
                break
            is_last = i + T >= n_total
            tv["first_frame_idx"] = i
            tv["frame_indices"] = torch.arange(i, min(i + T, n_total))

            if on_clip is not None:
                on_clip(i, targets)
            if shard is not None:
                if i + T > win_end:
                    win_start, win_end = i, i + self.num_frames_window_test
                    win_rows, win_pd = window_features_on_owner(model, x, list(range(win_start, min(win_end, n_total))), shard)
                out = sharded_clip_forward(model, targets, i, min(T, n_total - i), win_rows, win_pd, shard, device=x.device,
                                           lazy_masks=lazy_ok)
                if lazy_ok:
                    out, lazy = out
            else:
                if i + T > win_end:
                    win_start, win_end = i, i + self.num_frames_window_test
                    feats_window = model.backbone(x[win_start:win_end])
                    win_pd = None
                    head = model.sem_seg_head
                    if (self.pixel_decoder_once_per_window and self.num_frames_window_test > T and stride < T
                            and hasattr(head, "pixel_decoder") and hasattr(head, "predictor")):
                        mf, bfe, _enc, ms = head.pixel_decoder.forward_features(feats_window)
                        win_pd = (mf, bfe, list(ms))
                o = i - win_start
                if win_pd is not None:
                    mf, bfe, ms = win_pd
                    out = model.sem_seg_head.predictor([lv[o:o + T] for lv in ms], mf[o:o + T], bfe[o:o + T] if bfe is not None else None,
                                                       None, targets)
                else:
                    feats = {k: v[o:o + T] for k, v in feats_window.items()}
                    out = model.sem_seg_head(feats, targets=targets)
            out.pop("aux_outputs", None)

            out["pred_logits"] = out["pred_logits"].sigmoid()
            sl = self._class_slice(sub_task, tv["dataset_name"])
            if sl is not None:
                n_cls, start = sl
                assert start + n_cls <= out["pred_logits"].shape[-1]
                out["pred_logits"] = out["pred_logits"][..., start:start + n_cls]

            out = {k: v[0] for k, v in out.items() if v is not None}
            out = {k: v for k, v in out.items() if v is not None}
            out_learn = {k: v[: self.num_queries] for k, v in out.items()}
            out_prompt = {k: v[self.num_queries:] for k, v in out.items()}
            if lazy is not None:
                out_prompt["pred_masks"] = lazy.rows(torch.arange(self.num_queries, lazy.n_rows))
                out_learn.pop("pred_masks", None)

            if "vss" in sub_task:
                results.append(self.save_results_vss(i, out_learn, interim_size, image_size, out_size, is_last, stride))
                continue
            self.write_prompt_predictions_into_annotations_per_clip(i, out_prompt, targets, interim_size, image_size, stride)
            if i % self.detect_newly_interval_frames == 0 or tv["masks"].nelement() == 0:
                if "vis" in sub_task:
                    self.detect_newly_entities_per_clip_instance(out_learn, targets, interim_size, sharded=lazy)
                else:
                    self.detect_newly_entities_per_clip_pixel(out_learn, targets, interim_size)
                self.write_newly_entities_into_annotations_per_clip(i, out_learn, targets, interim_size)
            is_out = i > self.num_prev_frames_memory and i % self.num_frames_window_output == self.num_prev_frames_memory
            if is_out or is_last:
                save = self.save_results_vis if "vis" in sub_task else self.save_results_vps
                results.append(save(i, targets, interim_size, image_size, out_size, is_last))
                w = self.num_frames_window_output
                tv["mask_logits"] = tv["mask_logits"][:, w:]
                tv["masks"] = tv["masks"][:, w:]
                tv["occurrence"] = tv["occurrence"][:, w:]
            if not is_last and "masks" in tv:
                self.pad_zero_annotations_for_next_clip(targets, min(stride, video_len - i - T))
        if "vss" in sub_task:
            return self.vss_output_results(targets, results, out_size)
        if "vps" in sub_task:
            return self.vps_output_results(targets, results, out_size)
        if not merge_results:
            return results
        from .results import vis_clip_instances_to_coco_json_video
# ... 456 lines not shown
```

### univs_amd/layers.py

```python
import math
from typing import Optional

import torch
import torch.nn.functional as F
from torch import nn


def _as_fp32(v):
    if isinstance(v, torch.Tensor):
        return v.float() if v.is_floating_point() and v.dtype != torch.float32 else v
    if isinstance(v, (list, tuple)):
        return type(v)(_as_fp32(u) for u in v)
    if isinstance(v, dict):
        return {k: _as_fp32(u) for k, u in v.items()}
    return v


def fp32_region(fn):
    import functools
    import inspect
    names = list(inspect.signature(fn).parameters)[1:]

    @functools.wraps(fn)
    def wrapper(self, *args, **kwargs):
        if not torch.is_autocast_enabled("cuda"):
            return fn(self, *args, **kwargs)
        with torch.autocast(device_type="cuda", enabled=False):
            args = [a if (i < len(names) and names[i] == "targets") else _as_fp32(a) for i, a in enumerate(args)]
            return fn(self, *args, **{k: (v if k == "targets" else _as_fp32(v)) for k, v in kwargs.items()})
    return wrapper


from .switches import SWITCHES


class Conv2d(nn.Conv2d):

    def __init__(self, *args, **kwargs):
        norm = kwargs.pop("norm", None)
        activation = kwargs.pop("activation", None)
        super().__init__(*args, **kwargs)
        self.norm = norm
        self.activation = activation

    def convolve(self, x):
        y = None
        if (SWITCHES.split_conv and x.is_cuda and self.kernel_size == (1, 1) and self.stride == (1, 1) and self.padding == (0, 0)
                and self.dilation == (1, 1) and self.groups == 1):
            from . import ops
            y = ops.conv1x1(x, self.weight, self.bias)
        return y if y is not None else F.conv2d(x, self.weight, self.bias, self.stride, self.padding, self.dilation, self.groups)

    def forward(self, x):
        y = None
        if (SWITCHES.split_conv and x.is_cuda and self.bias is None and self.kernel_size == (3, 3) and self.stride == (1, 1)
                and self.padding == (1, 1) and self.dilation == (1, 1) and self.groups == 1):
            from . import ops
            y = ops.conv3x3(x, self.weight)
        elif (SWITCHES.split_conv and x.is_cuda and self.kernel_size == (1, 1) and self.stride == (1, 1) and self.padding == (0, 0)
              and self.dilation == (1, 1) and self.groups == 1):
            from . import ops
            y = ops.conv1x1(x, self.weight, self.bias)
        x = y if y is not None else F.conv2d(x, self.weight, self.bias, self.stride, self.padding, self.dilation, self.groups)
        if isinstance(self.norm, nn.GroupNorm) and x.dtype == torch.float32:
            from . import ops
            relu = self.activation is F.relu
            x = ops.group_norm(x, self.norm.num_groups, self.norm.weight, self.norm.bias, self.norm.eps, relu=relu)
            return x if relu or self.activation is None else self.activation(x)
        if self.norm is not None:
            x = self.norm(x)
        if self.activation is not None:
            x = self.activation(x)
        return x


def to_device_async(t, device):
    device = torch.device(device)
    if t.device == device:
        return t
    if device.type != "cuda" or t.is_cuda:
        return t.to(device)
    return t.pin_memory().to(device, non_blocking=True)


def get_norm(norm, out_channels):
    if norm is None or norm == "":
        return None
    if norm == "GN":
        return nn.GroupNorm(32, out_channels)
    if norm == "LN":
        return nn.LayerNorm(out_channels)
    raise ValueError(f"unsupported norm {norm!r}")


def point_sample(input, point_coords, **kwargs):
    add_dim = False
    if point_coords.dim() == 3:
        add_dim = True
        point_coords = point_coords.unsqueeze(2)
    output = F.grid_sample(input, 2.0 * point_coords - 1.0, **kwargs)
    if add_dim:
        output = output.squeeze(3)
    return output


class MultiheadAttention(nn.Module):

    def __init__(self, embed_dim, num_heads, dropout=0.0):
        super().__init__()
        assert embed_dim % num_heads == 0
        self.embed_dim, self.num_heads, self.head_dim = embed_dim, num_heads, embed_dim // num_heads
        self.in_proj_weight = nn.Parameter(torch.empty(3 * embed_dim, embed_dim))
        self.in_proj_bias = nn.Parameter(torch.zeros(3 * embed_dim))
        self.out_proj = nn.Linear(embed_dim, embed_dim)
        nn.init.xavier_uniform_(self.in_proj_weight)

# ... 27 lines not shown
        L, N, E = query.shape
        S = key.shape[0] if kv is None else kv[0].shape[0]
        h, d = self.num_heads, self.head_dim
        w, b = self.in_proj_weight, self.in_proj_bias
        small = query.is_cuda and _small(query, w, b)

        def lin(x, r0, n, add=None):
            if small and x.numel() // E <= 4096:
                from . import ops
                y = ops.small_linear(x, w, b, rows=(r0, n), x_add=add)
                if y is not None:
                    return y
            wr, br = self._packed_rows(r0, n)
            return linear(x if add is None else x + add, wr, br)
        if kv is not None:
            q = lin(query, 0, E, query_add)
            k, v = kv
        elif query is key and key is value and query_add is None:
            q, k, v = lin(query, 0, 3 * E).chunk(3, dim=-1)
        else:
            if query is key:
                qkv = None
                if small and query_add is not None and value is query and E % 32 == 0:
                    from . import ops
                    qkv = ops.small_linear(query, w, b, x_add=query_add, add_features=2 * E)
                if qkv is not None:
                    q, k, v = qkv.chunk(3, dim=-1)
                else:
                    q, k = lin(query, 0, 2 * E, query_add).chunk(2, dim=-1)
                    v = lin(value, 2 * E, E)
            else:
                q = lin(query, 0, E, query_add)
                if key is value:
                    k, v = lin(key, E, 2 * E).chunk(2, dim=-1)
                else:
                    k = lin(key, E, E)
                    v = lin(value, 2 * E, E)

        def project(out):
            if norm is None:
                y = linear(out, self.out_proj.weight, self.out_proj.bias)
                return y if residual is None else residual + y
            return linear_norm(out, self.out_proj, residual, norm)
        if (SWITCHES.fused_cross_attention and query.is_cuda and not need_weights and d == 32 and S >= 64 and L <= 2048
                and (attn_mask is None or (attn_mask.dtype in (torch.bool, torch.uint8)
                                           and ((attn_mask.dim() == 3 and attn_mask.shape[0] == N) or (attn_mask.dim() == 2 and N == 1))))):
            from . import ops
            m3 = attn_mask
            if isinstance(attn_mask, torch.Tensor):
                if S % 4:
                    m3 = ops.pad4_mask(attn_mask)
                if m3.dim() == 2:
                    m3 = m3.view(1, L, m3.shape[-1])
            out = ops.cross_attention(q, k, v, m3, h, 1.0 / math.sqrt(d))
            if out is not None:
                return project(out), None
        if attn_mask is not None and not isinstance(attn_mask, torch.Tensor):
            attn_mask = attn_mask.materialize()
        q = q.reshape(L, N, h, d).permute(1, 2, 0, 3)
        k = k.reshape(S, N, h, d).permute(1, 2, 0, 3)
        v = v.reshape(S, N, h, d).permute(1, 2, 0, 3)
        scores = torch.matmul(q * (1.0 / math.sqrt(d)), k.transpose(-1, -2))
        fused = attn_mask is None or (attn_mask.dtype in (torch.bool, torch.uint8)
                                      and (attn_mask.dim() == 2 or attn_mask.shape[0] == N))
        if fused:
            from . import ops
            if attn_mask is not None and attn_mask.dim() == 2:
                attn = ops.masked_softmax_(scores.view(1, N * h, L, S), attn_mask.view(1, L, S)).view(N, h, L, S)
            else:
                attn = ops.masked_softmax_(scores, attn_mask)
        else:
            m = attn_mask.view(N, h, L, S) if attn_mask.shape[0] == N * h else attn_mask.view(N, 1, L, S)
            scores = scores.masked_fill(m, float("-inf")) if m.dtype == torch.bool else scores + m
            attn = torch.softmax(scores, dim=-1)
        out = torch.matmul(attn, v)
        out = out.permute(2, 0, 1, 3).reshape(L, N, E)
        out = project(out)
        if need_weights:
            return out, (attn.mean(dim=1) if average_attn_weights else attn)
        return out, None


class MLP(nn.Module):

    def __init__(self, input_dim, hidden_dim, output_dim, num_layers):
        super().__init__()
        self.num_layers = num_layers
        h = [hidden_dim] * (num_layers - 1)
        self.layers = nn.ModuleList(nn.Linear(n, k) for n, k in zip([input_dim] + h, h + [output_dim]))

    def forward(self, x, transpose01=False, in_norm=None, want_normed=False):
        if (SWITCHES.small_mlp_chain and x.is_cuda and self.num_layers <= 3 and x.shape[-1] == 256 and not torch.is_grad_enabled()
                and x.numel() // 256 <= 4096 and (in_norm is None or SWITCHES.small_mlp_norm)):
            from . import ops
            chain = [(l_.weight, l_.bias, i < self.num_layers - 1) for i, l_ in enumerate(self.layers)]
            r = ops.small_mlp(x, chain, in_ln=None if in_norm is None else (in_norm.weight, in_norm.bias, in_norm.eps),
                              want_normed=want_normed, transpose01=transpose01)
            if r is not None:
                return r
        xn = None
        if in_norm is not None:
            x = xn = in_norm(x)
        y = self._forward_layers(x, transpose01)
        return (y, xn) if want_normed else y

    def _forward_layers(self, x, transpose01):
# ... 107 lines not shown
```

### univs_amd/modeling/backbone/swin.py

```python

import numpy as np
import torch
import torch.nn.functional as F
from torch import nn

from ... import ops
from ...layers import fp32_region, layer_norm
from ...registry import BACKBONE_REGISTRY, ShapeSpec


def _to_2tuple(x):
    return tuple(x) if isinstance(x, (tuple, list)) else (x, x)


from ...switches import SWITCHES


def _linear(mod, x):
    y = ops.linear_fused(x, mod.weight, mod.bias) if (SWITCHES.swin_fused_linear and (SWITCHES.swin_fused_parts & 1) and x.is_cuda) else None
    return y if y is not None else mod(x)


class Mlp(nn.Module):
    def __init__(self, in_features, hidden_features=None, out_features=None):
# ... 264 lines not shown
                 ape=False, patch_norm=True, out_indices=(0, 1, 2, 3)):
        super().__init__()
        self.pretrain_img_size = pretrain_img_size
        self.num_layers = len(depths)
        self.embed_dim, self.ape, self.patch_norm, self.out_indices = embed_dim, ape, patch_norm, out_indices
        self.patch_embed = PatchEmbed(patch_size, in_chans, embed_dim, patch_norm)
        if self.ape:
            pis, ps = _to_2tuple(pretrain_img_size), _to_2tuple(patch_size)
            self.absolute_pos_embed = nn.Parameter(torch.zeros(1, embed_dim, pis[0] // ps[0], pis[1] // ps[1]))
        self.layers = nn.ModuleList()
        for i in range(self.num_layers):
            self.layers.append(BasicLayer(int(embed_dim * 2 ** i), depths[i], num_heads[i], window_size,
                                          mlp_ratio, qkv_bias, qk_scale,
                                          PatchMerging if (i < self.num_layers - 1) else None))
        self.num_features = [int(embed_dim * 2 ** i) for i in range(self.num_layers)]
        for i in out_indices:
            self.add_module(f"norm{i}", nn.LayerNorm(self.num_features[i]))

    @fp32_region
    def forward(self, x):
        if SWITCHES.graphs and x.is_cuda and not self.training:
            g = self.__dict__.get("_graphed")
            if g is None:
                from ...graphs import GraphedCallable
                g = self.__dict__["_graphed"] = GraphedCallable(self._forward)
            return g(x)
        return self._forward(x)

    def set_attention_mma(self, mma):
        if mma not in ops.MMA_DTYPES:
            raise ValueError(f"set_attention_mma: {mma!r} (one of {sorted(ops.MMA_DTYPES)})")
        for m in self.modules():
            if isinstance(m, WindowAttention):
                m.mma = mma
        self._graphed = None
        return self

    def _forward(self, x):
        if self.ape:
            x = self.patch_embed(x)
            Wh, Ww = x.size(2), x.size(3)
            ape = F.interpolate(self.absolute_pos_embed, size=(Wh, Ww), mode="bicubic")
            x = (x + ape).flatten(2).transpose(1, 2)
        else:
            x, Wh, Ww = self.patch_embed.tokens(x)
        outs = {}
        for i in range(self.num_layers):
            if i in self.out_indices and x.is_cuda and not torch.is_grad_enabled():
                x_out, H, W, x, Wh, Ww, x_normed = self.layers[i](x, Wh, Ww, out_norm=getattr(self, f"norm{i}"))
            else:
                (x_out, H, W, x, Wh, Ww), x_normed = self.layers[i](x, Wh, Ww), None
            if i in self.out_indices:
                x_out = x_normed if x_normed is not None else layer_norm(getattr(self, f"norm{i}"), x_out)
                outs[f"res{i + 2}"] = ops.transpose_last2(x_out).view(-1, self.num_features[i], H, W)
        return outs


@BACKBONE_REGISTRY.register()
class D2SwinTransformer(SwinTransformer):

    def __init__(self, cfg, input_shape=None):
        s = cfg.MODEL.SWIN
        super().__init__(s.PRETRAIN_IMG_SIZE, s.PATCH_SIZE, 3, s.EMBED_DIM, s.DEPTHS, s.NUM_HEADS,
                         s.WINDOW_SIZE, s.MLP_RATIO, s.QKV_BIAS, s.QK_SCALE, s.APE, s.PATCH_NORM)
        self._out_features = s.OUT_FEATURES
        self._out_feature_strides = {"res2": 4, "res3": 8, "res4": 16, "res5": 32}
        self._out_feature_channels = {f"res{i + 2}": self.num_features[i] for i in range(4)}

    def forward(self, x):
        assert x.dim() == 4, f"SwinTransformer takes an input of shape (N, C, H, W). Got {x.shape} instead!"
        y = super().forward(x)
        return {k: v for k, v in y.items() if k in self._out_features}

    def output_shape(self):
        return {name: ShapeSpec(channels=self._out_feature_channels[name],
                                stride=self._out_feature_strides[name]) for name in self._out_features}

    @property
    def size_divisibility(self):
        return 32
```

### univs_amd/modeling/meta_arch/mask_former_head.py

```python
from typing import Dict

from torch import nn

from ...registry import SEM_SEG_HEADS_REGISTRY, TRANSFORMER_DECODER_REGISTRY, ShapeSpec, configurable


def build_pixel_decoder(cfg, input_shape):
    name = cfg.MODEL.SEM_SEG_HEAD.PIXEL_DECODER_NAME
    model = SEM_SEG_HEADS_REGISTRY.get(name)(cfg, input_shape)
    if not callable(getattr(model, "forward_features", None)):
        raise ValueError("Only SEM_SEG_HEADS with forward_features method can be used as pixel decoder. "
                         f"Please implement forward_features for {name} to only return mask features.")
    return model


def build_transformer_decoder(cfg, in_channels, mask_classification=True):
    name = cfg.MODEL.MASK_FORMER.TRANSFORMER_DECODER_NAME
    return TRANSFORMER_DECODER_REGISTRY.get(name)(cfg, in_channels, mask_classification)


@SEM_SEG_HEADS_REGISTRY.register()
class MaskFormerHead(nn.Module):
    _version = 2

    @configurable
    def __init__(self, input_shape: Dict[str, ShapeSpec], *, num_classes: int, pixel_decoder: nn.Module,
                 pixel_decoder_name: str, loss_weight: float = 1.0, ignore_value: int = -1,
                 transformer_predictor: nn.Module, transformer_in_feature: str, frozen_pixel_decoder: bool = False,
                 frozen_mask_convs: bool = False, frozen_predictor: bool = False):
        super().__init__()
        input_shape = sorted(input_shape.items(), key=lambda x: x[1].stride)
        self.in_features = [k for k, v in input_shape]
        self.ignore_value = ignore_value
        self.common_stride = 4
        self.loss_weight = loss_weight
        self.pixel_decoder = pixel_decoder
        self.pixel_decoder_name = pixel_decoder_name
        self.predictor = transformer_predictor
        self.transformer_in_feature = transformer_in_feature
        self.num_classes = num_classes

    @classmethod
    def from_config(cls, cfg, input_shape: Dict[str, ShapeSpec]):
        tif = cfg.MODEL.MASK_FORMER.TRANSFORMER_IN_FEATURE
        if tif in ("transformer_encoder", "multi_scale_pixel_decoder"):
            in_ch = cfg.MODEL.SEM_SEG_HEAD.CONVS_DIM
        elif tif == "pixel_embedding":
            in_ch = cfg.MODEL.SEM_SEG_HEAD.MASK_DIM
        else:
            in_ch = input_shape[tif].channels
        return {
            "input_shape": {k: v for k, v in input_shape.items() if k in cfg.MODEL.SEM_SEG_HEAD.IN_FEATURES},
            "ignore_value": cfg.MODEL.SEM_SEG_HEAD.IGNORE_VALUE,
            "num_classes": cfg.MODEL.SEM_SEG_HEAD.NUM_CLASSES,
            "pixel_decoder": build_pixel_decoder(cfg, input_shape),
            "pixel_decoder_name": cfg.MODEL.SEM_SEG_HEAD.PIXEL_DECODER_NAME,
            "loss_weight": cfg.MODEL.SEM_SEG_HEAD.LOSS_WEIGHT,
            "transformer_in_feature": tif,
            "transformer_predictor": build_transformer_decoder(cfg, in_ch, mask_classification=True),
            "frozen_pixel_decoder": cfg.MODEL.SEM_SEG_HEAD.FROZEN_PIXEL_DECODER,
            "frozen_mask_convs": cfg.MODEL.SEM_SEG_HEAD.FROZEN_MASK_CONVS,
            "frozen_predictor": cfg.MODEL.SEM_SEG_HEAD.FROZEN_PREDICTOR,
        }

    def forward(self, features, mask=None, targets=None):
        return self.layers(features, mask, targets)

    def prefetch_prompts(self, targets, num_frames):
        if targets is not None and hasattr(self.predictor, "prefetch_prompts"):
            self.predictor.prefetch_prompts(targets, num_frames)

    def layers(self, features, mask=None, targets=None):
        if self.pixel_decoder_name != "MSDeformAttnPixelDecoder":
            raise ValueError(f"pixel decoder {self.pixel_decoder_name} is outside the hot path (SURVEY.md section 2)")
        if targets is not None and hasattr(self.predictor, "prefetch_prompts"):
            self.predictor.prefetch_prompts(targets, next(iter(features.values())).shape[0])
        mask_features, mask_features_bfe_conv, enc_features, multi_scale_features = \
            self.pixel_decoder.forward_features(features)
        if self.transformer_in_feature != "multi_scale_pixel_decoder":
            raise ValueError("only TRANSFORMER_IN_FEATURE='multi_scale_pixel_decoder' is on the hot path")
        return self.predictor(multi_scale_features, mask_features, mask_features_bfe_conv, mask, targets)
```

### univs_amd/modeling/pixel_decoder/msdeformattn.py

```python
from typing import Callable, Dict, List, Optional, Union

import numpy as np
import torch
import torch.nn.functional as F
from torch import nn

from ... import ops
from ...layers import Conv2d, get_activation_fn, get_norm, layer_norm, linear, linear_act
from ...registry import SEM_SEG_HEADS_REGISTRY, ShapeSpec, configurable
from ..position_encoding import PositionEmbeddingSine


from ...switches import SWITCHES


def _shape_list(spatial_shapes):
    return spatial_shapes.tolist() if isinstance(spatial_shapes, torch.Tensor) else list(spatial_shapes)


class MSDeformAttn(nn.Module):
    def __init__(self, d_model=256, n_levels=4, n_heads=8, n_points=4):
        super().__init__()
        if d_model % n_heads != 0:
            raise ValueError(f"d_model must be divisible by n_heads, but got {d_model} and {n_heads}")
        self.im2col_step = 128
        self.d_model, self.n_levels, self.n_heads, self.n_points = d_model, n_levels, n_heads, n_points
        self.sampling_offsets = nn.Linear(d_model, n_heads * n_levels * n_points * 2)
        self.attention_weights = nn.Linear(d_model, n_heads * n_levels * n_points)
        self.value_proj = nn.Linear(d_model, d_model)
        self.output_proj = nn.Linear(d_model, d_model)

    def _merged_query_proj(self):
        so, aw = self.sampling_offsets, self.attention_weights
        key = (so.weight.data_ptr(), so.weight._version, aw.weight.data_ptr(), aw.weight._version,
               so.bias._version, aw.bias._version, so.weight.device)
        c = getattr(self, "_qproj_cache", None)
        if c is None or c[0] != key:
            with torch.no_grad():
                c = (key, torch.cat([so.weight, aw.weight]).contiguous(), torch.cat([so.bias, aw.bias]).contiguous())
            self._qproj_cache = c
        return c[1], c[2], so.weight.shape[0]

    def _head_major_query_proj(self, order):
        so, aw = self.sampling_offsets, self.attention_weights
        key = (so.weight.data_ptr(), so.weight._version, aw.weight.data_ptr(), aw.weight._version,
               so.bias._version, aw.bias._version, so.weight.device, order)
        c = getattr(self, "_qproj_hm_cache", None)
        if c is None or c[0] != key:
            M, L, P = self.n_heads, self.n_levels, self.n_points
            n_off = M * L * P * 2
            idx = []
            for m in range(M):
                for p in range(P):
                    idx += [((m * L + l) * P + p) * 2 + xy for l in order for xy in (0, 1)]
                    idx += [n_off + (m * L + l) * P + p for l in order]
            with torch.no_grad():
                ix = torch.tensor(idx, dtype=torch.long, device=so.weight.device)
                w = torch.cat([so.weight, aw.weight])[ix].contiguous()
                b = torch.cat([so.bias, aw.bias])[ix].contiguous()
            c = (key, w, b)
# ... 214 lines not shown
        chans = transformer_in_channels[::-1] if self.transformer_num_feature_levels > 1 else [transformer_in_channels[-1]]
        self.input_proj = nn.ModuleList([
            nn.Sequential(nn.Conv2d(c, conv_dim, kernel_size=1), nn.GroupNorm(32, conv_dim)) for c in chans])
        self.transformer = MSDeformAttnTransformerEncoderOnly(
            d_model=conv_dim, dropout=transformer_dropout, nhead=transformer_nheads,
            dim_feedforward=transformer_dim_feedforward, num_encoder_layers=transformer_enc_layers,
            num_feature_levels=self.transformer_num_feature_levels)
        self.pe_layer = PositionEmbeddingSine(conv_dim // 2, normalize=True)
        self.mask_dim = mask_dim
        self.mask_features = Conv2d(conv_dim, mask_dim, kernel_size=1, stride=1, padding=0)
        self.maskformer_num_feature_levels = 3
        self.common_stride = common_stride
        stride = min(self.transformer_feature_strides)
        self.num_fpn_levels = int(np.log2(stride) - np.log2(self.common_stride))
        lateral_convs, output_convs = [], []
        use_bias = norm == ""
        for idx, in_channels in enumerate(self.feature_channels[:self.num_fpn_levels]):
            lateral_conv = Conv2d(in_channels, conv_dim, kernel_size=1, bias=use_bias, norm=get_norm(norm, conv_dim))
            output_conv = Conv2d(conv_dim, conv_dim, kernel_size=3, stride=1, padding=1, bias=use_bias,
                                 norm=get_norm(norm, conv_dim), activation=F.relu)
            self.add_module(f"adapter_{idx + 1}", lateral_conv)
            self.add_module(f"layer_{idx + 1}", output_conv)
            lateral_convs.append(lateral_conv)
            output_convs.append(output_conv)
        self.lateral_convs = lateral_convs[::-1]
        self.output_convs = output_convs[::-1]
        self._pe_cache = {}

    @classmethod
    def from_config(cls, cfg, input_shape: Dict[str, ShapeSpec]):
        ret = {}
        ret["input_shape"] = {k: v for k, v in input_shape.items() if k in cfg.MODEL.SEM_SEG_HEAD.IN_FEATURES}
        ret["conv_dim"] = cfg.MODEL.SEM_SEG_HEAD.CONVS_DIM
        ret["mask_dim"] = cfg.MODEL.SEM_SEG_HEAD.MASK_DIM
        ret["norm"] = cfg.MODEL.SEM_SEG_HEAD.NORM
        ret["transformer_dropout"] = cfg.MODEL.MASK_FORMER.DROPOUT
        ret["transformer_nheads"] = cfg.MODEL.MASK_FORMER.NHEADS
        ret["transformer_dim_feedforward"] = 1024
        ret["transformer_enc_layers"] = cfg.MODEL.SEM_SEG_HEAD.TRANSFORMER_ENC_LAYERS
        ret["transformer_in_features"] = cfg.MODEL.SEM_SEG_HEAD.DEFORMABLE_TRANSFORMER_ENCODER_IN_FEATURES
        ret["common_stride"] = cfg.MODEL.SEM_SEG_HEAD.COMMON_STRIDE
        return ret

    def _pos(self, x):
        key = (tuple(x.shape[-2:]), str(x.device))
        p = self._pe_cache.get(key)
        if p is None:
            if len(self._pe_cache) > 16:
                self._pe_cache.clear()
            p = self.pe_layer(x[:1])
            self._pe_cache[key] = p
        return p

    def forward_features(self, features):
        with torch.autocast(device_type=next(iter(features.values())).device.type, enabled=False):
            if SWITCHES.graphs and not self.training and all(f.is_cuda for f in features.values()):
                g = self.__dict__.get("_graphed")
                if g is None:
                    from ...graphs import GraphedCallable
                    g = self.__dict__["_graphed"] = GraphedCallable(self._forward_features)
                return g({k: features[k] for k in self.in_features})
            return self._forward_features(features)

    def _input_proj(self, idx, x):
        conv, gn = self.input_proj[idx][0], self.input_proj[idx][1]
        if x.is_cuda and x.dtype == torch.float32 and not ops.needs_grad(x, conv.weight):
            y = ops.conv1x1(x, conv.weight, conv.bias) if SWITCHES.split_conv else None
            if y is None:
                y = conv(x)
            return ops.group_norm(y, gn.num_groups, gn.weight, gn.bias, gn.eps)
        return self.input_proj[idx](x)

    def _forward_features(self, features):
        srcs, pos, affines = [], [], []
        for idx, f in enumerate(self.transformer_in_features[::-1]):
            x = features[f].float()
            conv, gn = self.input_proj[idx][0], self.input_proj[idx][1]
            if x.is_cuda and not torch.is_grad_enabled() and not ops.needs_grad(x, conv.weight):
                raw = ops.conv1x1(x, conv.weight, conv.bias) if SWITCHES.split_conv else None
                raw = conv(x) if raw is None else raw
                srcs.append(raw)
                affines.append(ops.group_norm_affine(raw, gn.num_groups, gn.weight, gn.bias, gn.eps))
            else:
                srcs.append(self._input_proj(idx, x))
                affines.append(None)
            pos.append(self._pos(x))
        if all(a is None for a in affines):
            y, spatial_shapes, level_start_index = self.transformer(srcs, pos)
        else:
            y, spatial_shapes, level_start_index = self.transformer(srcs, pos, affines)
        bs = y.shape[0]
        sizes = [h * w for (h, w) in spatial_shapes]
        y = torch.split(y, sizes, dim=1)
        if y[0].is_cuda:
            out = [ops.transpose_last2(z).view(bs, -1, spatial_shapes[i][0], spatial_shapes[i][1]) for i, z in enumerate(y)]
        else:
            out = [z.transpose(1, 2).reshape(bs, -1, spatial_shapes[i][0], spatial_shapes[i][1]) for i, z in enumerate(y)]
        for idx, f in enumerate(self.in_features[:self.num_fpn_levels][::-1]):
            x = features[f].float()
            lat = self.lateral_convs[idx]
            y_ = None
            if (x.is_cuda and isinstance(lat.norm, nn.GroupNorm) and lat.activation is None and not torch.is_grad_enabled()
                    and x.shape[-2] == 2 * out[-1].shape[-2] and x.shape[-1] == 2 * out[-1].shape[-1]):
                raw = lat.convolve(x)
                y_ = ops.upsample2x_add(out[-1], raw, ops.group_norm_affine(raw, lat.norm.num_groups, lat.norm.weight, lat.norm.bias,
                                                                          lat.norm.eps))
                if y_ is None:
                    cur_fpn = ops.group_norm(raw, lat.norm.num_groups, lat.norm.weight, lat.norm.bias, lat.norm.eps)
                    y_ = ops.bilinear_resample(out[-1], cur_fpn.shape[-2:], addend=cur_fpn)
            if y_ is None:
                cur_fpn = lat(x)
                y_ = ops.bilinear_resample(out[-1], cur_fpn.shape[-2:], addend=cur_fpn)
            out.append(self.output_convs[idx](y_))
        multi_scale_features = out[:self.maskformer_num_feature_levels]
        return self.mask_features(out[-1]), out[-1], out[0], multi_scale_features
```

### univs_amd/ops.py

```python
import contextlib
import weakref
import ctypes
import math
import os

import torch

from . import _lib
from .switches import SWITCHES

_raw_stream = torch._C._cuda_getCurrentRawStream


def _stream_ptr(t):
    return _raw_stream(t.device.index if t.device.index is not None else torch.cuda.current_device())


def _ptr(t):
    return t.data_ptr()


def _opt(t, offset=0):
    return None if t is None else t.data_ptr() + offset

# ... 725 lines not shown
        if tuple(shift_mask.shape) != (nW, n, n):
            raise RuntimeError("window_attention_image: bad shift_mask shape")
    else:
        shift_mask = None
    if qkv_bias is not None:
        _require_gpu("window_attention_image", qkv_bias)
        if qkv_bias.numel() != 3 * nH * hd:
            raise RuntimeError("window_attention_image: bad qkv_bias shape")
    out = torch.empty((B, L, nH * hd), dtype=torch.float32, device=qkv.device)
    _call("window_attention_image", _lib.load().univs_window_attention_image_mma, qkv, _ptr(qkv), _opt(qkv_bias), _ptr(bias), _opt(shift_mask),
          B, int(H), int(W), ws, int(shift), nH, hd, float(scale), MMA_DTYPES[mma], _ptr(out), uncovered="raise")
    return out


def masked_softmax_(scores, mask=None):
    _inference_only("masked_softmax_", scores)
    _require_gpu("masked_softmax_", scores)
    if scores.dtype != torch.float32 or scores.dim() != 4:
        raise RuntimeError("masked_softmax_: float32 [N, h, L, S] only")
    N, h, L, S = scores.shape
    if mask is not None:
        _require_gpu("masked_softmax_", mask)
        if tuple(mask.shape) != (N, L, S) or mask.dtype not in (torch.bool, torch.uint8):
            raise RuntimeError("masked_softmax_: mask must be bool / uint8 [N, L, S]")
    _call("masked_softmax_", _lib.load().univs_masked_softmax_f32, scores, _ptr(scores), _opt(mask), N, h, L, S, uncovered="raise")
    return scores


def _seq_first_ld(t, N, E):
    if t.stride(-1) != 1 or t.dim() != 3:
        return None
    ld = t.stride(1) if N > 1 else (t.stride(0) if t.shape[0] > 1 else E)
    if ld < E or ld % 4 or (t.shape[0] > 1 and t.stride(0) != N * ld) or (t.data_ptr() & 15):
        return None
    return ld


_PAD4 = {}


def pad4_mask(mask):
    if mask.shape[-1] % 4 == 0:
        return mask.contiguous()
    hit = _PAD4.get(id(mask))
    if hit is not None and hit[0]() is mask and hit[1] == mask._version:
        return hit[2]
    padded = torch.nn.functional.pad(mask, (0, (-mask.shape[-1]) % 4)).contiguous()
    if len(_PAD4) > 32:
        _PAD4.clear()
    _PAD4[id(mask)] = (weakref.ref(mask), mask._version, padded)
    return padded


def cross_attention(q, k, v, mask, num_heads, scale):
    _inference_only("cross_attention", q, k, v)
    if not (q.is_cuda and q.dtype == torch.float32 and k.dtype == torch.float32 and v.dtype == torch.float32):
        return None
    L, N, E = q.shape
    S = k.shape[0]
    H = int(num_heads)
    if E != 32 * H or tuple(k.shape) != (S, N, E) or tuple(v.shape) != (S, N, E) or S < 32 or N * H > 65535 or L < 1:
        return None
    flags, gen = None, 0
    if isinstance(mask, DeferredMask):
        if tuple(mask.shape) != (N, L, S) or S % 4 != 0:
            return None
        if mask._bool is not None:
            mask = mask._bool.view(torch.uint8)
        else:
            mask.check_fresh()
            mask, flags, gen = mask.mask, mask.flags, mask.gen
    elif mask is not None:
        if tuple(mask.shape) not in ((N, L, S), (N, L, (S + 3) & ~3)) or mask.dtype not in (torch.bool, torch.uint8) or not mask.is_cuda:
            return None
        mask = pad4_mask(mask) if mask.shape[-1] % 4 else mask.contiguous()
    lds_ = []
    for t in (q, k, v):
        ld = _seq_first_ld(t, N, E)
        if ld is None:
            t = t.contiguous()
            ld = E
        lds_.append((t, ld))
    (q, ldq), (k, ldk), (v, ldv) = lds_
    lib = _lib.load()
    ws = torch.empty(int(lib.univs_cross_attention_workspace(L, S, N, H)), dtype=torch.float32, device=q.device)
    out = torch.empty((L, N, E), dtype=torch.float32, device=q.device)
    ok = _call("cross_attention", lib.univs_cross_attention_flagged_f32, q, _ptr(q), _ptr(k), _ptr(v), _opt(mask), _opt(flags), gen,
               L, S, N, H, 32, ldq, ldk, ldv, float(scale), _ptr(ws), _ptr(out))
    return out if ok else None


def proca_attention(qkv0, kd, vd, num_heads):
    _inference_only("proca_attention", qkv0, kd, vd)
    _require_gpu("proca_attention", qkv0, kd, vd)
    Qp, L, T, E = kd.shape
    h = int(num_heads)
    if (any(t.dtype != torch.float32 or not t.is_contiguous() for t in (qkv0, kd, vd)) or tuple(vd.shape) != tuple(kd.shape)
            or tuple(qkv0.shape) != (Qp * T, 3 * E) or E % h):
        raise RuntimeError("proca_attention: contiguous float32 qkv0 [Q_p T, 3 E], kd / vd [Q_p, L, T, E]")
    out = torch.empty((Qp * T, E), dtype=torch.float32, device=kd.device)
    ok = _call("proca_attention", _lib.load().univs_proca_attention_f32, kd, _ptr(qkv0), _ptr(kd), _ptr(vd), Qp, L, T, h, E // h,
               1.0 / math.sqrt(E // h), _ptr(out))
    return out if ok else None


def layer_norm(x, weight, bias, eps=1e-5, residual=None, return_sum=False, post_add=None):
    x, weight, bias = x.contiguous(), weight.contiguous(), bias.contiguous()
    _inference_only("layer_norm", x, weight, bias, residual)
    _require_gpu("layer_norm", x, weight, bias)
    if x.dtype != torch.float32:
        raise RuntimeError("layer_norm: float32 only")
    if return_sum and residual is None:
        raise RuntimeError("layer_norm: return_sum needs a residual")
    C = x.shape[-1]
    if tuple(weight.shape) != (C,) or tuple(bias.shape) != (C,):
        raise RuntimeError("layer_norm: weight / bias must be [C]")
    if residual is not None:
        residual = residual.contiguous()
        _require_gpu("layer_norm", residual)
        if residual.shape != x.shape or residual.dtype != torch.float32:
            raise RuntimeError("layer_norm: residual must match x")
    out = torch.empty_like(x)
    s = torch.empty_like(x) if return_sum else None
    rows = x.numel() // max(C, 1)
    if post_add is not None:
        if residual is None or return_sum:
            raise RuntimeError("layer_norm: post_add needs a residual and excludes return_sum")
        post_add = post_add.contiguous()
        _require_gpu("layer_norm", post_add)
        arows = post_add.numel() // max(C, 1)
        lead = x.dim() - post_add.dim()
        ok = (post_add.dtype == torch.float32 and lead >= 0 and post_add.shape[-1] == C and rows % max(arows, 1) == 0
              and all(a == b or (i < post_add.dim() - 1 and all(int(d) == 1 for d in post_add.shape[:i + 1]))
                      for i, (a, b) in enumerate(zip(post_add.shape, x.shape[lead:]))))
        if not ok:
            raise RuntimeError("layer_norm: post_add must match x or broadcast over its leading dimensions")
        out2 = torch.empty_like(x)
        _call("layer_norm", _lib.load().univs_layer_norm_add_f32, x, _ptr(x), _ptr(residual), _ptr(weight), _ptr(bias), _ptr(post_add), arows,
              rows, C, float(eps), None, _ptr(out), _ptr(out2), uncovered="raise")
# ... 542 lines not shown
```

### univs_amd/switches.py

```python
import contextlib
import dataclasses
import os


def _flag(name, default):
    v = os.environ.get(name)
    return default if v is None or v == "" else v != "0"


@dataclasses.dataclass
class Switches:
    msda_strips: bool = True
    msda_heads: bool = True
    split_linear: bool = True
    split_conv: bool = True
    swin_fused_linear: bool = True
    swin_fused_parts: int = 7
    fused_mlp: bool = True
    fused_mlp_max_c: int = 256
    fused_norm1: bool = True
    small_linear: bool = True
    fused_cross_attention: bool = True
    linear_kmax: int = 4096
    presplit_kmin: int = 768
    small_mlp_chain: bool = True
    fused_proca: bool = True
    fused_sampler: bool = True
    small_mlp_norm: bool = True
    resident_presplit: bool = True
    sampler: str = "auto"
    graphs: bool = False


SWITCHES = Switches(
    msda_strips=_flag("UNIVS_MSDA_STRIPS", True), msda_heads=_flag("UNIVS_MSDA_HEADS", True), split_linear=_flag("UNIVS_SPLIT_LINEAR", True),
    split_conv=_flag("UNIVS_SPLIT_CONV", True), swin_fused_linear=_flag("UNIVS_SWIN_FUSED_LINEAR", True),
    swin_fused_parts=int(os.environ.get("UNIVS_SWIN_FUSED_PARTS", "7")), linear_kmax=int(os.environ.get("UNIVS_LINEAR_KMAX", "4096")),
    sampler=os.environ.get("UNIVS_SAMPLER", "auto"), graphs=_flag("UNIVS_GRAPHS", False),
    presplit_kmin=int(os.environ.get("UNIVS_PRESPLIT_KMIN", "768")), fused_mlp=_flag("UNIVS_FUSED_MLP", True),
    fused_cross_attention=_flag("UNIVS_FUSED_XATTN", True), fused_norm1=_flag("UNIVS_FUSED_NORM1", True), small_linear=_flag("UNIVS_SMALL_LINEAR", True),
    resident_presplit=_flag("UNIVS_RESIDENT_PRESPLIT", True), small_mlp_chain=_flag("UNIVS_SMALL_MLP_CHAIN", True), fused_proca=_flag("UNIVS_FUSED_PROCA", True),
    fused_sampler=_flag("UNIVS_FUSED_SAMPLER", True), small_mlp_norm=_flag("UNIVS_SMALL_MLP_NORM", True))
if SWITCHES.sampler not in ("auto", "reference", "device"):
    raise ValueError(f"UNIVS_SAMPLER={SWITCHES.sampler!r} (expected 'auto', 'reference' or 'device')")


@contextlib.contextmanager
def override(**kw):
    old = {k: getattr(SWITCHES, k) for k in kw}
    for k, v in kw.items():
        if not hasattr(SWITCHES, k):
            raise KeyError(k)
        setattr(SWITCHES, k, v)
    try:
        yield SWITCHES
    finally:
        for k, v in old.items():
            setattr(SWITCHES, k, v)
```

Measured before the change: 364.5 frames/s.

## Fuse GroupNorm affine into 1x1 conv GEMM and consume channels-last features directly

Adds a fused 1x1 conv kernel that applies a per-frame GroupNorm affine (with ReLU) to its input while streaming it. The last FPN output conv's norm is folded into the mask_features projection, so the normalized tensor is not materialized. Lateral and input-projection convs can also read channels-last backbone features in place instead of transposing them first. It also splits cross-attention into a partials stage and a merge that can be fused into the following small linear (off by default). The cost is more template variants and extra shape-coverage conditions that fall back to the old paths.

```diff
diff --git a/include/univs_fused_hip.h b/include/univs_fused_hip.h
--- /dev/null
+++ b/include/univs_fused_hip.h
@@ -0,0 +1,26 @@
+#ifndef UNIVS_FUSED_HIP_H
+#define UNIVS_FUSED_HIP_H
+
+#include <stdint.h>
+
+#include "univs_hip.h"
+
+#ifdef __cplusplus
+extern "C" {
+#endif
+
+int univs_conv1x1_fused_presplit_f32(const float* x, int channels_last, const float* affine, const void* wp, const float* winv,
+                                     const float* bias, int T, int Cin, int Cout, int H, int W, float* y, void* stream);
+
+int univs_cross_attention_partials_f32(const float* q, const float* k, const float* v, const uint8_t* mask, const uint32_t* mask_row_flags,
+                                       uint32_t mask_generation, int L, int S, int N, int H, int head_dim, int ldq, int ldk, int ldv,
+                                       float scale, float* workspace, int* plan, void* stream);
+
+int univs_small_linear_merged_presplit_f32(const float* workspace, long long workspace_floats, int plan, int L, int N, int H, const void* wp,
+                                           const float* winv, const float* bias, int n_w, int f_off, const float* residual,
+                                           const float* ln_weight, const float* ln_bias, float ln_eps, int n_out, float* y, void* stream);
+
+#ifdef __cplusplus
+}
+#endif
+#endif
diff --git a/univs_amd/_lib.py b/univs_amd/_lib.py
--- a/univs_amd/_lib.py
+++ b/univs_amd/_lib.py
@@ -58,6 +58,9 @@
 EVAL_HEADER_PATH = os.path.join(_HERE, "..", "include", "univs_eval_hip.h")
 with open(EVAL_HEADER_PATH) as _f:
     EVAL_SIGNATURES = parse_signatures(_f.read())
+FUSED_HEADER_PATH = os.path.join(_HERE, "..", "include", "univs_fused_hip.h")
+with open(FUSED_HEADER_PATH) as _f:
+    FUSED_SIGNATURES = parse_signatures(_f.read())
 
 _lib = None
 
@@ -75,7 +78,7 @@
             f"{LIB_PATH} not found: the HIP extension is mandatory (no CPU fallback). "
             "Build it with `python -m univs_amd.build`.")
     lib = ctypes.CDLL(LIB_PATH)
-    for name, (res, args) in (*SIGNATURES.items(), *EVAL_SIGNATURES.items()):
+    for name, (res, args) in (*SIGNATURES.items(), *EVAL_SIGNATURES.items(), *FUSED_SIGNATURES.items()):
         fn = getattr(lib, name)
         fn.restype = res
         fn.argtypes = args
diff --git a/univs_amd/build.py b/univs_amd/build.py
--- a/univs_amd/build.py
+++ b/univs_amd/build.py
@@ -8,8 +8,8 @@
 LIB = os.path.join(HERE, "libunivs_hip.so")
 SOURCES = ["capi.hip", "msda_fwd.hip", "msda_tiled2.hip", "msda_strips.hip", "msda_heads.hip", "msda_bwd.hip", "msda_prepare.hip", "mask_decode.hip", "linear_split.hip", "linear_f16x3.hip", "gemm_f16x3_stream.hip", "gemm_f16x3_tile.hip", "mlp_f16x3.hip", "small_linear.hip", "cross_attn.hip", "window_attn.hip", "window_attn_f16.hip", "resample.hip", "semantic_extract.hip", "layer_norm.hip", "group_norm.hip", "softmax.hip", "proca_attn.hip", "prompt_sampler.hip", "transpose.hip", "mask_stats.hip", "image_post.hip", "video_post.hip", "pair_count.hip", "vss_count.hip", "davis_count.hip", "vis_overlap.hip"]
 HEADERS = [os.path.join(CSRC, "common.h"), os.path.join(CSRC, "msda_common.h"), os.path.join(CSRC, "msda_geometry.h"), os.path.join(CSRC, "msda_dev.h"), os.path.join(CSRC, "msda_window_geom.h"), os.path.join(CSRC, "msda_strips_geom.h"), os.path.join(CSRC, "msda_heads_geom.h"), os.path.join(CSRC, "config.h"), os.path.join(CSRC, "window_attn.h"), os.path.join(CSRC, "f16x3.h"), os.path.join(CSRC, "gemm_plan.h"), os.path.join(CSRC, "resample_taps.h"),
-           os.path.join(CSRC, "mask_post.h"), os.path.join(CSRC, "count_core.h"), os.path.join(CSRC, "launchers.h"), os.path.join(HERE, "..", "include", "univs_hip.h"),
-           os.path.join(HERE, "..", "include", "univs_eval_hip.h")]
+           os.path.join(CSRC, "mask_post.h"), os.path.join(CSRC, "count_core.h"), os.path.join(CSRC, "launchers.h"), os.path.join(CSRC, "xattn_merge.h"), os.path.join(HERE, "..", "include", "univs_hip.h"),
+           os.path.join(HERE, "..", "include", "univs_eval_hip.h"), os.path.join(HERE, "..", "include", "univs_fused_hip.h")]
 
 
 def _hipcc():
diff --git a/univs_amd/csrc/capi.hip b/univs_amd/csrc/capi.hip
--- a/univs_amd/csrc/capi.hip
+++ b/univs_amd/csrc/capi.hip
@@ -4,6 +4,7 @@
 #include <mutex>
 
 #include "../../include/univs_eval_hip.h"
+#include "../../include/univs_fused_hip.h"
 #include "common.h"
 #include "config.h"
 #include "launchers.h"
@@ -300,6 +301,49 @@
   const Entry e("univs_conv3x3_nhwc_presplit_f32", stream);
   return conv_entry(e, "Cin % 128, Cout % 16, >= 4096 pixels", T, Cin, Cout, H, W, x && wp && winv && y,
                     [&] { return conv3x3_nhwc_f16x3_f32(x, wp, winv, y, T, Cin, Cout, H, W, e.st); });
+}
+
+int univs_conv1x1_fused_presplit_f32(const float* x, int channels_last, const float* affine, const void* wp, const float* winv,
+                                     const float* bias, int T, int Cin, int Cout, int H, int W, float* y, void* stream) {
+  const Entry e("univs_conv1x1_fused_presplit_f32", stream);
+  return conv_entry(e, "Cin % 96 or % 128, Cout % 16, >= 4096 pixels; with an affine H W >= 256 and Cin <= 1024", T, Cin, Cout, H, W,
+                    x && wp && winv && y,
+                    [&] { return conv1x1_fused_f16x3_f32(x, channels_last, affine, wp, winv, bias, y, T, Cin, Cout, H, W, e.st); });
+}
+
+int univs_cross_attention_partials_f32(const float* q, const float* k, const float* v, const uint8_t* mask, const uint32_t* mask_row_flags,
+                                       uint32_t mask_generation, int L, int S, int N, int H, int head_dim, int ldq, int ldk, int ldv,
+                                       float scale, float* workspace, int* plan, void* stream) {
+  const Entry e("univs_cross_attention_partials_f32", stream);
+  if (!plan) return e.invalid("NULL plan (a host int)");
+  *plan = 0;
+  if (L < 0 || S < 1 || N < 0 || H < 1 || head_dim < 1) return e.invalid("bad dimensions L=%d S=%d N=%d H=%d head_dim=%d", L, S, N, H, head_dim);
+  if (L == 0 || N == 0) return UNIVS_OK;
+  if (!q || !k || !v || !workspace || (mask_row_flags && !mask)) return e.invalid("NULL data pointer (row flags come with a mask)");
+  return e.covered(cross_attention_partials_f32(q, k, v, mask, mask_row_flags, mask_generation, L, S, N, H, head_dim, ldq, ldk, ldv, scale,
+                                                workspace, plan, e.st),
+                   "L=%d S=%d N=%d H=%d head_dim=%d not covered (head_dim == 32, S >= 32, with a mask S %% 4 == 0, "
+                   "N * H <= 65535, 16-byte aligned pointers)", L, S, N, H, head_dim);
+}
+
+int univs_small_linear_merged_presplit_f32(const float* workspace, long long workspace_floats, int plan, int L, int N, int H, const void* wp,
+                                           const float* winv, const float* bias, int n_w, int f_off, const float* residual,
+                                           const float* ln_weight, const float* ln_bias, float ln_eps, int n_out, float* y, void* stream) {
+  const Entry e("univs_small_linear_merged_presplit_f32", stream);
+  const int nseg = plan & 0xffff, nqb = plan >> 16;
+  if (L < 0 || N < 0 || H < 1 || n_out < 0 || n_w < 1 || f_off < 0 || f_off + n_out > n_w)
+    return e.invalid("bad arguments L=%d N=%d H=%d n_out=%d n_w=%d f_off=%d", L, N, H, n_out, n_w, f_off);
+  if (L == 0 || N == 0 || n_out == 0) return UNIVS_OK;
+  if (plan <= 0 || nseg < 1 || nqb < 1 || nqb > 7) return e.invalid("plan=%d is not segments + 65536 * query blocks per wave (1 .. 7)", plan);
+  const long long chunks = ((long long)L + 16 * nqb - 1) / (16 * nqb);
+  const long long need = chunks * N * H * nseg * (16 * nqb) * 34;
+  if (workspace_floats < need)
+    return e.invalid("workspace of %lld floats, the plan %d of L=%d N=%d H=%d takes %lld", workspace_floats, plan, L, N, H, need);
+  if (!workspace || !wp || !winv || !y || (ln_bias && !ln_weight)) return e.null_pointer();
+  return e.covered(small_linear_merged_f32(workspace, plan, L, N, H, wp, winv, bias, n_w, f_off, residual, ln_weight, ln_bias, ln_eps, y,
+                                           n_out, e.st),
+                   "L=%d N=%d H=%d n_out=%d not covered (H <= 8, n_out %% 16 == 0, f_off %% 4 == 0, with a LayerNorm n_out == 256, "
+                   "L N <= 1 048 560, 16-byte aligned pointers)", L, N, H, n_out);
 }
 
 int univs_patch_embed4_f32(const float* x, const float* weight, const float* bias, const float* ln_weight, const float* ln_bias, float ln_eps,
diff --git a/univs_amd/csrc/cross_attn.hip b/univs_amd/csrc/cross_attn.hip
--- a/univs_amd/csrc/cross_attn.hip
+++ b/univs_amd/csrc/cross_attn.hip
@@ -1,5 +1,6 @@
 #include "common.h"
 #include "launchers.h"
+#include "xattn_merge.h"
 #include "config.h"
 #include "f16x3.h"
 
@@ -25,7 +26,6 @@
   float qscale;
 };
 
-constexpr int XA_PART = 34;
 #ifndef UNIVS_XA_VS
 #define UNIVS_XA_VS 36
 #endif
@@ -384,17 +384,9 @@
   const int chunk = q / Lp, ql = q - chunk * Lp;
   const float* base = ws + ((((long long)chunk * N * H + nh) * nseg) * Lp + ql) * XA_PART;
   const long long pstride = (long long)Lp * XA_PART;
-  float M = -INFINITY;
-#pragma unroll 8
-  for (int p = 0; p < nseg; ++p) M = fmaxf(M, base[p * pstride + 32]);
-  float acc = 0.f, l = 0.f;
-#pragma unroll 8
-  for (int p = 0; p < nseg; ++p) {
-    const float f = __builtin_amdgcn_exp2f(base[p * pstride + 32] - M);
-    acc = fmaf(base[p * pstride + c], f, acc);
-    l = fmaf(base[p * pstride + 33], f, l);
-  }
-  out[((long long)q * N + n) * (H * 32) + h * 32 + c] = acc / l;
+  float r[1];
+  xa_merge_partials<1>(base, pstride, nseg, c, r);
+  out[((long long)q * N + n) * (H * 32) + h * 32 + c] = r[0];
 }
 
 constexpr int XA_MAX_NQB = 7;
@@ -432,12 +424,13 @@
   return (size_t)nchunks * N * H * p.nseg * (16 * p.nqb) * XA_PART;
 }
 
-int cross_attention_f32(const float* q, const float* k, const float* v, const unsigned char* mask, const unsigned* row_flags,
-                        unsigned generation, int L, int S, int N, int H, int hd, int ldq, int ldk, int ldv, float scale, float* ws,
-                        float* out, hipStream_t st) {
+int cross_attention_partials_f32(const float* q, const float* k, const float* v, const unsigned char* mask, const unsigned* row_flags,
+                                 unsigned generation, int L, int S, int N, int H, int hd, int ldq, int ldk, int ldv, float scale, float* ws,
+                                 int* plan_out, hipStream_t st) {
+  if (plan_out) *plan_out = 0;
   if (L <= 0 || N <= 0 || H <= 0) return UNIVS_OK;
   auto mis = [](const void* p) { return (reinterpret_cast<uintptr_t>(p) & 15) != 0; };
-  if (hd != 32 || S < 32 || (mask && ((row_flags && S % 4 != 0) || (reinterpret_cast<uintptr_t>(mask) & 3))) || mis(q) || mis(k) || mis(v) || mis(out) ||
+  if (hd != 32 || S < 32 || (mask && ((row_flags && S % 4 != 0) || (reinterpret_cast<uintptr_t>(mask) & 3))) || mis(q) || mis(k) || mis(v) ||
       mis(ws) || (long long)N * H > 65535)
     return UNIVS_ERR_NOT_IMPLEMENTED;
   const XaPlan plan = xa_plan(L, S, N, H);
@@ -452,7 +445,7 @@
   a.mask = mask;
   a.flags = mask ? row_flags : nullptr;
   a.gen = generation;
-  a.ws = ws; a.out = out;
+  a.ws = ws; a.out = nullptr;
   a.L = L; a.S = S; a.N = N; a.H = H; a.nseg = nseg;
   a.Lfull = L; a.l0 = 0;
   a.ldq = ldq; a.ldk = ldk; a.ldv = ldv;
@@ -467,8 +460,19 @@
     case 6: hipLaunchKernelGGL(xattn_partial<6>, grid, dim3(64), 0, st, a); break;
     default: hipLaunchKernelGGL(xattn_partial<7>, grid, dim3(64), 0, st, a); break;
   }
-  int rc = check_launch("xattn_partial");
+  if (plan_out) *plan_out = nseg + 65536 * nqb;
+  return check_launch("xattn_partial");
+}
+
+int cross_attention_f32(const float* q, const float* k, const float* v, const unsigned char* mask, const unsigned* row_flags,
+                        unsigned generation, int L, int S, int N, int H, int hd, int ldq, int ldk, int ldv, float scale, float* ws,
+                        float* out, hipStream_t st) {
+  if (L <= 0 || N <= 0 || H <= 0) return UNIVS_OK;
+  if (reinterpret_cast<uintptr_t>(out) & 15) return UNIVS_ERR_NOT_IMPLEMENTED;
+  int plan = 0;
+  const int rc = cross_attention_partials_f32(q, k, v, mask, row_flags, generation, L, S, N, H, hd, ldq, ldk, ldv, scale, ws, &plan, st);
   if (rc != UNIVS_OK) return rc;
+  const int nseg = plan & 0xffff, nqb = plan >> 16;
   const long long total = (long long)N * H * L * 32;
   hipLaunchKernelGGL(xattn_merge, dim3((unsigned)((total + 255) / 256)), dim3(256), 0, st, ws, out, L, 16 * nqb, N, H, nseg);
   return check_launch("xattn_merge");
diff --git a/univs_amd/csrc/gemm_f16x3_stream.hip b/univs_amd/csrc/gemm_f16x3_stream.hip
--- a/univs_amd/csrc/gemm_f16x3_stream.hip
+++ b/univs_amd/csrc/gemm_f16x3_stream.hip
@@ -65,9 +65,10 @@
   int Cin, Cout, H, Wd, HW;
   int tap0;
   int remap;
+  const float* affine;
 };
 
-template <int RB, int RING, int XMODE>
+template <int RB, int RING, int XMODE, bool AFF = false>
 __global__ __launch_bounds__(GS_THREADS, 512 / GS_THREADS) void gemm_f16x3_stream(const GsArgs a) {
   extern __shared__ __attribute__((aligned(16))) u32x4 Wst[];
   [[maybe_unused]] const int gts = UNIVS_GT_SLOT();
@@ -90,6 +91,7 @@
   const int j = lane & 15, g = lane >> 4;
   float* bias_lds = reinterpret_cast<float*>(Wst + 2 * SLAB);
   float* winv_lds = bias_lds + Rp;
+  [[maybe_unused]] float* aff_lds = winv_lds + Rp;
   constexpr int NWV = GS_THREADS / 64;
 
   const int WT = (M + GS_TILE_M - 1) / GS_TILE_M;
@@ -138,6 +140,7 @@
   struct TileRows {
     unsigned vo[2];
     int py[2], px[2];
+    unsigned ao[2];
   };
   auto tile_rows = [&](int tt, TileRows& t) __attribute__((always_inline)) {
 #pragma unroll
@@ -146,16 +149,19 @@
       if (XMODE == 0) {
         t.vo[c] = ((unsigned)m * (unsigned)K + (unsigned)(8 * g)) * 4u;
         t.py[c] = t.px[c] = 0;
+        t.ao[c] = 0u;
       } else if (XMODE == 2) {
         const int f = m / a.HW, rem = m - f * a.HW;
-        t.py[c] = rem / a.Wd;
-        t.px[c] = rem - t.py[c] * a.Wd;
+        t.py[c] = AFF ? 0 : rem / a.Wd;
+        t.px[c] = AFF ? 0 : rem - t.py[c] * a.Wd;
         t.vo[c] = ((unsigned)m * (unsigned)a.Cin + (unsigned)(8 * g)) * 4u;
+        t.ao[c] = (unsigned)(((f & 1) * a.Cin + 8 * g) * 8);
       } else {
         const int f = m / a.HW, rem = m - f * a.HW;
-        t.py[c] = rem / a.Wd;
-        t.px[c] = rem - t.py[c] * a.Wd;
+        t.py[c] = AFF ? 0 : rem / a.Wd;
+        t.px[c] = AFF ? 0 : rem - t.py[c] * a.Wd;
         t.vo[c] = (unsigned)((f * a.Cin + 8 * g) * a.HW + rem) * 4u;
+        t.ao[c] = (unsigned)(((f & 1) * a.Cin + 8 * g) * 8);
       }
     }
   };
@@ -174,7 +180,7 @@
       const int dy = tap / 3 - 1, dx = tap - (tap / 3) * 3 - 1;
 #pragma unroll
       for (int c = 0; c < 2; ++c) {
-        const bool inb = (unsigned)(t.py[c] + dy) < (unsigned)a.H && (unsigned)(t.px[c] + dx) < (unsigned)a.Wd;
+        const bool inb = AFF || ((unsigned)(t.py[c] + dy) < (unsigned)a.H && (unsigned)(t.px[c] + dx) < (unsigned)a.Wd);
         const unsigned vo = inb ? t.vo[c] + (unsigned)((dy * a.Wd + dx) * a.Cin * 4) : 0xFFFFFFE0u;
         buf[c][0] = __builtin_bit_cast(f32x4, __builtin_amdgcn_raw_buffer_load_b128(xrs, vo, cb * 4, 0));
         buf[c][1] = __builtin_bit_cast(f32x4, __builtin_amdgcn_raw_buffer_load_b128(xrs, vo + 16u, cb * 4, 0));
@@ -185,7 +191,7 @@
       const int dy = tap / 3 - 1, dx = tap - (tap / 3) * 3 - 1;
 #pragma unroll
       for (int c = 0; c < 2; ++c) {
-        const bool inb = (unsigned)(t.py[c] + dy) < (unsigned)a.H && (unsigned)(t.px[c] + dx) < (unsigned)a.Wd;
+        const bool inb = AFF || ((unsigned)(t.py[c] + dy) < (unsigned)a.H && (unsigned)(t.px[c] + dx) < (unsigned)a.Wd);
         const unsigned vo = inb ? t.vo[c] + (unsigned)((dy * a.Wd + dx) * 4) : 0xFFFFFFF0u;
 #pragma unroll
         for (int e = 0; e < 8; ++e)
@@ -236,10 +242,25 @@
   UNIVS_GT(g_gs_trace, gts, 2);
   UNIVS_GT_VAL(g_gs_trace, gts, 63, rounds);
   int gq = 0;
+  [[maybe_unused]] int aff_f0 = -1, aff_f1 = -1;
 #pragma unroll 1
   for (int rd = 0; rd < rounds; ++rd) {
     const int tt = wg0 + rd * NWV + wave;
     const bool tile_ok = tt < wg1;
+    if constexpr (AFF) {
+      const int r0 = min((wg0 + rd * NWV) * GS_TILE_M, M - 1), r1 = min(r0 + NWV * GS_TILE_M - 1, M - 1);
+      const int f0 = r0 / a.HW, f1 = r1 / a.HW;
+      if (f0 != aff_f0 || f1 != aff_f1) {
+        __syncthreads();
+        const int n = (f1 - f0 + 1) * a.Cin;
+        for (int i = tid; i < n; i += GS_THREADS) {
+          const int f = i < a.Cin ? f0 : f1, ch = i < a.Cin ? i : i - a.Cin;
+          *reinterpret_cast<float2*>(aff_lds + ((f & 1) * a.Cin + ch) * 2) = *reinterpret_cast<const float2*>(a.affine + ((size_t)f * a.Cin + ch) * 2);
+        }
+        aff_f0 = f0;
+        aff_f1 = f1;
+      }
+    }
 #pragma unroll
     for (int rb = 0; rb < RB; ++rb) acc[rb][0] = acc[rb][1] = (f32x4){0.f, 0.f, 0.f, 0.f};
     eset[0] = eset[1] = -1000;
@@ -254,6 +275,22 @@
 #pragma unroll
       for (int u = 0; u < RING; ++u) {
         if (u > 0) w_commit(bufc ^ 1, u - 1);
+        if constexpr (AFF) {
+          const unsigned kb = (unsigned)((q * RING + u) * 32 * 8);
+#pragma unroll
+          for (int c = 0; c < 2; ++c) {
+            const f32x4* ap = reinterpret_cast<const f32x4*>(reinterpret_cast<const char*>(aff_lds) + t_cur.ao[c] + kb);
+#pragma unroll
+            for (int h = 0; h < 2; ++h) {
+              const f32x4 p0 = ap[2 * h], p1 = ap[2 * h + 1];
+              raw[u][c][h][0] = fmaxf(fma_single(raw[u][c][h][0], p0[0], p0[1]), 0.f);
+              raw[u][c][h][1] = fmaxf(fma_single(raw[u][c][h][1], p0[2], p0[3]), 0.f);
+              raw[u][c][h][2] = fmaxf(fma_single(raw[u][c][h][2], p1[0], p1[1]), 0.f);
+              raw[u][c][h][3] = fmaxf(fma_single(raw[u][c][h][3], p1[2], p1[3]), 0.f);
+            }
+            __builtin_amdgcn_sched_barrier(0);
+          }
+        }
         bool need = false;
         int enew[2];
 #pragma unroll
@@ -371,20 +408,23 @@
   UNIVS_GT_REAL(g_gs_trace, gts, 61);
 }
 
-template <int XMODE>
+template <int XMODE, bool AFF = false>
 static int gs_launch(const GsArgs& a0, hipStream_t st) {
   GsArgs a = a0;
   const StreamPlan p = plan_stream(XMODE, a.M, a.N, a.K, cu_count(), config());
   a.rows_per_pass = p.rows_per_pass;
   a.remap = p.remap;
   const int RB = p.RB, ring = p.ring;
-  const size_t lds = p.lds;
+  const size_t lds = p.lds + (AFF ? gs_affine_lds(a.Cin) : 0);
+  if (AFF && !stream_affine_plan_covered(RB, ring)) return UNIVS_ERR_NOT_IMPLEMENTED;
   dim3 grid(p.gx, p.passes), block(GS_THREADS);
 #define UNIVS_GS(rb, rg)                                                                                          \
   do {                                                                                                            \
-    (void)hipFuncSetAttribute(reinterpret_cast<const void*>(&gemm_f16x3_stream<rb, rg, XMODE>),                   \
-                              hipFuncAttributeMaxDynamicSharedMemorySize, (int)lds);                              \
-    hipLaunchKernelGGL((gemm_f16x3_stream<rb, rg, XMODE>), grid, block, lds, st, a);                              \
+    if constexpr (!AFF || stream_affine_plan_covered(rb, rg)) {                                                   \
+      (void)hipFuncSetAttribute(reinterpret_cast<const void*>(&gemm_f16x3_stream<rb, rg, XMODE, AFF>),            \
+                                hipFuncAttributeMaxDynamicSharedMemorySize, (int)lds);                            \
+      hipLaunchKernelGGL((gemm_f16x3_stream<rb, rg, XMODE, AFF>), grid, block, lds, st, a);                       \
+    }                                                                                                             \
   } while (0)
 #define UNIVS_GS_RB(rb)                    \
   case rb:                                 \
@@ -420,16 +460,19 @@
 
 template <int XMODE>
 static int gs_conv(const float* x, const void* wp, const float* winv, const float* bias, float* y, int T, int Cin, int Cout, int H, int W,
-                   int taps, hipStream_t st) {
+                   int taps, hipStream_t st, const float* affine = nullptr) {
   if (T <= 0 || Cout <= 0 || H <= 0 || W <= 0) return UNIVS_OK;
   const long long M = (long long)T * H * W;
   if (!stream_conv_covered(M, Cin, Cout, taps) || !aligned16(x, wp, y, winv, bias)) return UNIVS_ERR_NOT_IMPLEMENTED;
+  if (affine && (taps != 1 || !stream_affine_covered((long long)H * W, Cin) || (reinterpret_cast<uintptr_t>(affine) & 7)))
+    return UNIVS_ERR_NOT_IMPLEMENTED;
   GsArgs a{};
   a.X = x; a.Wp = reinterpret_cast<const u32x4*>(wp); a.winv = winv; a.bias = bias; a.Res = nullptr; a.Y = y;
   a.M = (int)M; a.N = Cout; a.K = taps * Cin; a.epi = GS_EPI_NONE;
   a.Cin = Cin; a.Cout = Cout; a.H = H; a.Wd = W; a.HW = H * W;
   a.tap0 = taps == 9 ? 0 : 4;
-  return gs_launch<XMODE>(a, st);
+  a.affine = affine;
+  return affine ? gs_launch<XMODE, true>(a, st) : gs_launch<XMODE>(a, st);
 }
 
 int conv3x3_f16x3_f32(const float* x, const void* wp, const float* winv, float* y, int T, int Cin, int Cout, int H, int W,
@@ -445,6 +488,12 @@
 int conv1x1_f16x3_f32(const float* x, const void* wp, const float* winv, const float* bias, float* y, int T, int Cin, int Cout, int H,
                       int W, hipStream_t st) {
   return gs_conv<1>(x, wp, winv, bias, y, T, Cin, Cout, H, W, 1, st);
+}
+
+int conv1x1_fused_f16x3_f32(const float* x, int channels_last, const float* affine, const void* wp, const float* winv, const float* bias,
+                            float* y, int T, int Cin, int Cout, int H, int W, hipStream_t st) {
+  return channels_last ? gs_conv<2>(x, wp, winv, bias, y, T, Cin, Cout, H, W, 1, st, affine)
+                       : gs_conv<1>(x, wp, winv, bias, y, T, Cin, Cout, H, W, 1, st, affine);
 }
 
 }
diff --git a/univs_amd/csrc/gemm_plan.h b/univs_amd/csrc/gemm_plan.h
--- a/univs_amd/csrc/gemm_plan.h
+++ b/univs_amd/csrc/gemm_plan.h
@@ -112,6 +112,9 @@
 inline bool stream_conv_covered(long long M, int Cin, int Cout, int taps) {
   return (taps == 9 ? Cin % 128 == 0 : k_ring(Cin) != 0) && Cout % 16 == 0 && M >= 4096 && fits_int32(M, std::max(Cin, Cout));
 }
+inline size_t gs_affine_lds(int Cin) { return (size_t)2 * Cin * 8; }
+inline bool stream_affine_covered(long long HW, int Cin) { return HW >= (GS_THREADS / 64) * GS_TILE_M && Cin <= 1024; }
+constexpr bool stream_affine_plan_covered(int RB, int ring) { return RB <= 4 || (RB == 8 && ring == 4); }
 struct StreamPlan {
   int RB, ring;
   unsigned gx, passes;
diff --git a/univs_amd/csrc/launchers.h b/univs_amd/csrc/launchers.h
--- a/univs_amd/csrc/launchers.h
+++ b/univs_amd/csrc/launchers.h
@@ -50,6 +50,8 @@
                       hipStream_t st);
 int conv1x1_f16x3_f32(const float* x, const void* wp, const float* winv, const float* bias, float* y, int T, int Cin, int Cout, int H,
                       int W, hipStream_t st);
+int conv1x1_fused_f16x3_f32(const float* x, int channels_last, const float* affine, const void* wp, const float* winv, const float* bias,
+                            float* y, int T, int Cin, int Cout, int H, int W, hipStream_t st);
 
 int linear_f16x3_tile_f32(const float* x, const void* wp, const float* winv, const float* bias, const float* residual, float* y,
                           long long M, int N, int K, int epi, hipStream_t st);
@@ -64,10 +66,16 @@
 int small_linear_f32(const float* x, const float* xadd, const void* wp, const float* winv, const float* bias, int n_w, int f_off,
                      const float* residual, const float* ln_g, const float* ln_b, float ln_eps, float* y, long long M, int N, int K,
                      int relu, int add_features, int out_T, hipStream_t st);
+int small_linear_merged_f32(const float* ws, int plan, int L, int Nb, int Hh, const void* wp, const float* winv, const float* bias, int n_w,
+                            int f_off, const float* residual, const float* ln_g, const float* ln_b, float ln_eps, float* y, int N,
+                            hipStream_t st);
 
 int cross_attention_f32(const float* q, const float* k, const float* v, const unsigned char* mask, const unsigned* row_flags,
                         unsigned generation, int L, int S, int N, int H, int hd, int ldq, int ldk, int ldv, float scale, float* ws,
                         float* out, hipStream_t st);
+int cross_attention_partials_f32(const float* q, const float* k, const float* v, const unsigned char* mask, const unsigned* row_flags,
+                                 unsigned generation, int L, int S, int N, int H, int hd, int ldq, int ldk, int ldv, float scale, float* ws,
+                                 int* plan_out, hipStream_t st);
 size_t cross_attention_workspace_floats(int L, int S, int N, int H);
 
 int window_attention_image_f32(const float* qkv, const float* qkv_bias, const float* bias, const float* shift_mask,
diff --git a/univs_amd/csrc/small_linear.hip b/univs_amd/csrc/small_linear.hip
--- a/univs_amd/csrc/small_linear.hip
+++ b/univs_amd/csrc/small_linear.hip
@@ -1,6 +1,7 @@
 #include "common.h"
 #include "f16x3.h"
 #include "launchers.h"
+#include "xattn_merge.h"
 
 #include <algorithm>
 #include <cstdlib>
@@ -25,6 +26,8 @@
   int M, N, K, Nw, f_off, relu;
   int out_T;
   int add_features;
+  const float* ws;
+  int nseg, Lp, Nb, Hh;
 };
 
 typedef unsigned sl_u2 __attribute__((ext_vector_type(2)));
@@ -35,7 +38,8 @@
   return __uint_as_float(s2.x) + __uint_as_float(s2.y);
 }
 
-__global__ __launch_bounds__(64 * SL_WAVES, 3) void small_linear_kernel(const SlArgs a) {
+template <bool MERGE>
+__global__ __launch_bounds__(64 * SL_WAVES, MERGE ? 2 : 3) void small_linear_kernel(const SlArgs a) {
   extern __shared__ __attribute__((aligned(16))) u32x4 xs[];
   __shared__ float red[2][SL_WAVES][16];
   __shared__ unsigned rmax[2][16];
@@ -79,8 +83,18 @@
     if (s_ < KS * 64) {
       const int ks = s_ >> 6, l_ = s_ & 63, j_ = l_ & 15, g_ = l_ >> 4;
       const long long off = (long long)min(row0 + j_, M - 1) * K + 32 * ks + 8 * g_;
-      xv[i][0] = *reinterpret_cast<const f32x4*>(a.X + off);
-      xv[i][1] = *reinterpret_cast<const f32x4*>(a.X + off + 4);
+      if constexpr (MERGE) {
+        const int r = min(row0 + j_, M - 1), q = r / a.Nb, n = r - q * a.Nb;
+        const int chunk = q / a.Lp, ql = q - chunk * a.Lp;
+        const float* base = a.ws + ((((long long)chunk * a.Nb * a.Hh + (n * a.Hh + ks)) * a.nseg) * a.Lp + ql) * XA_PART;
+        float mv[8];
+        xa_merge_partials<8>(base, (long long)a.Lp * XA_PART, a.nseg, 8 * g_, mv);
+        xv[i][0] = (f32x4){mv[0], mv[1], mv[2], mv[3]};
+        xv[i][1] = (f32x4){mv[4], mv[5], mv[6], mv[7]};
+      } else {
+        xv[i][0] = *reinterpret_cast<const f32x4*>(a.X + off);
+        xv[i][1] = *reinterpret_cast<const f32x4*>(a.X + off + 4);
+      }
       if (need_add) {
         xw[i][0] = xv[i][0] + *reinterpret_cast<const f32x4*>(a.Xadd + off);
         xw[i][1] = xv[i][1] + *reinterpret_cast<const f32x4*>(a.Xadd + off + 4);
@@ -221,8 +235,30 @@
   a.M = (int)M; a.N = N; a.K = K; a.Nw = n_w; a.f_off = f_off; a.relu = relu ? 1 : 0; a.add_features = add_features; a.out_T = out_T;
   dim3 grid((unsigned)((M + 15) / 16), (unsigned)((N + 32 * SL_WAVES - 1) / (32 * SL_WAVES)));
   const size_t lds = (size_t)2 * 2 * (K / 32) * 64 * 16;
-  hipLaunchKernelGGL(small_linear_kernel, grid, dim3(64 * SL_WAVES), lds, st, a);
+  hipLaunchKernelGGL(small_linear_kernel<false>, grid, dim3(64 * SL_WAVES), lds, st, a);
   return check_launch("small_linear_f32");
+}
+
+int small_linear_merged_f32(const float* ws, int plan, int L, int Nb, int Hh, const void* wp, const float* winv, const float* bias, int n_w,
+                            int f_off, const float* residual, const float* ln_g, const float* ln_b, float ln_eps, float* y, int N,
+                            hipStream_t st) {
+  const long long M = (long long)L * Nb;
+  if (M <= 0 || N <= 0) return UNIVS_OK;
+  auto mis = [](const void* p) { return (reinterpret_cast<uintptr_t>(p) & 15) != 0; };
+  const int nseg = plan & 0xffff, nqb = plan >> 16, K = 32 * Hh;
+  if (nseg < 1 || nqb < 1 || nqb > 7 || Hh < 1 || K > SL_KMAX || N % 16 != 0 || n_w % 4 != 0 || f_off % 4 != 0 || f_off < 0 || f_off + N > n_w ||
+      M > 16LL * 65535 || (ln_g && N != 32 * SL_WAVES) || (ln_b && !ln_g) || (reinterpret_cast<uintptr_t>(ws) & 7) || mis(wp) || mis(winv) ||
+      mis(bias) || mis(residual) || mis(ln_g) || mis(ln_b) || mis(y) || M * (long long)std::max(N, K) * 4 >= 0x7FFFFFFFLL)
+    return UNIVS_ERR_NOT_IMPLEMENTED;
+  SlArgs a{};
+  a.X = nullptr; a.Xadd = nullptr; a.Wp = reinterpret_cast<const u32x4*>(wp); a.winv = winv; a.bias = bias; a.Res = residual;
+  a.ln_g = ln_g; a.ln_b = ln_b; a.ln_eps = ln_eps; a.Y = y;
+  a.M = (int)M; a.N = N; a.K = K; a.Nw = n_w; a.f_off = f_off; a.relu = 0; a.add_features = 0; a.out_T = 0;
+  a.ws = ws; a.nseg = nseg; a.Lp = 16 * nqb; a.Nb = Nb; a.Hh = Hh;
+  dim3 grid((unsigned)((M + 15) / 16), (unsigned)((N + 32 * SL_WAVES - 1) / (32 * SL_WAVES)));
+  const size_t lds = (size_t)2 * 2 * (K / 32) * 64 * 16;
+  hipLaunchKernelGGL(small_linear_kernel<true>, grid, dim3(64 * SL_WAVES), lds, st, a);
+  return check_launch("small_linear_merged_f32");
 }
 
 struct SlChainArgs {
diff --git a/univs_amd/csrc/xattn_merge.h b/univs_amd/csrc/xattn_merge.h
--- /dev/null
+++ b/univs_amd/csrc/xattn_merge.h
@@ -0,0 +1,27 @@
+#pragma once
+#include <hip/hip_runtime.h>
+
+namespace univs {
+
+constexpr int XA_PART = 34;
+
+template <int NC>
+__device__ __forceinline__ void xa_merge_partials(const float* __restrict__ base, long long pstride, int nseg, int c0, float (&out)[NC]) {
+  float M = -INFINITY;
+#pragma unroll 8
+  for (int p = 0; p < nseg; ++p) M = fmaxf(M, base[p * pstride + 32]);
+  float acc[NC], l = 0.f;
+#pragma unroll
+  for (int e = 0; e < NC; ++e) acc[e] = 0.f;
+#pragma unroll(NC == 1 ? 8 : 4)
+  for (int p = 0; p < nseg; ++p) {
+    const float f = __builtin_amdgcn_exp2f(base[p * pstride + 32] - M);
+#pragma unroll
+    for (int e = 0; e < NC; ++e) acc[e] = fmaf(base[p * pstride + c0 + e], f, acc[e]);
+    l = fmaf(base[p * pstride + 33], f, l);
+  }
+#pragma unroll
+  for (int e = 0; e < NC; ++e) out[e] = acc[e] / l;
+}
+
+}
diff --git a/univs_amd/fused_ops.py b/univs_amd/fused_ops.py
--- /dev/null
+++ b/univs_amd/fused_ops.py
@@ -0,0 +1,73 @@
+import ctypes
+
+import torch
+
+from . import _lib, ops
+from .switches import SWITCHES
+
+
+def conv1x1_fused(x, weight, bias=None, affine=None):
+    name = "conv1x1_fused"
+    for t in (x, weight, bias, affine):
+        if t is not None and not t.is_cuda:
+            raise ops._cpu_refusal(name, f"tensor on {t.device}")
+    ops._inference_only(name, x, weight, bias, affine)
+    if (x.dtype != torch.float32 or weight.dtype != torch.float32 or x.dim() != 4 or weight.dim() != 4 or tuple(weight.shape[2:]) != (1, 1)
+            or weight.shape[1] != x.shape[1] or SWITCHES.presplit_kmin <= 0):
+        return None
+    T, Cin, H, W = (int(v) for v in x.shape)
+    Cout = int(weight.shape[0])
+    if x.is_contiguous():
+        channels_last = 0
+    elif x.is_contiguous(memory_format=torch.channels_last):
+        channels_last = 1
+    else:
+        return None
+    if bias is not None and (bias.dtype != torch.float32 or tuple(bias.shape) != (Cout,) or not bias.is_contiguous()):
+        return None
+    if affine is not None and (affine.dtype != torch.float32 or tuple(affine.shape) != (T * Cin, 2) or not affine.is_contiguous()):
+        raise RuntimeError(f"{name}: affine must be contiguous float32 [T * Cin, 2] = {(T * Cin, 2)}, got {affine.dtype} {tuple(affine.shape)}")
+    y = torch.empty((T, Cout, H, W), dtype=torch.float32, device=x.device)
+    wp, winv = ops.presplit_weights(weight)
+    ok = ops._call(name, _lib.load().univs_conv1x1_fused_presplit_f32, x, ops._ptr(x), channels_last, ops._opt(affine), ops._ptr(wp),
+                   ops._ptr(winv), ops._opt(bias), T, Cin, Cout, H, W, ops._ptr(y))
+    return y if ok else None
+
+
+def attention_out_proj(q, k, v, mask, num_heads, scale, weight, bias=None, residual=None, ln=None):
+    name = "attention_out_proj"
+    for t in (q, k, v, weight, bias, residual):
+        if t is not None and not t.is_cuda:
+            raise ops._cpu_refusal(name, f"tensor on {t.device}")
+    ops._inference_only(name, q, k, v, weight, bias, residual)
+    args = ops._cross_attention_args(q, k, v, mask, num_heads)
+    if args is None or weight.dtype != torch.float32 or weight.dim() != 2:
+        return None
+    q, k, v, mask, flags, gen, L, S, N, H, ldq, ldk, ldv = args
+    Nw, M = int(weight.shape[0]), L * N
+    if weight.shape[1] != 32 * H or 32 * H > ops.SMALL_LINEAR_MAX_K or M > ops.SMALL_LINEAR_MAX_ROWS or Nw % 16 != 0 or (ln is not None and Nw != 256):
+        return None
+    r = None
+    if residual is not None:
+        if residual.dtype != torch.float32 or residual.numel() != M * Nw or residual.shape[-1] != Nw:
+            return None
+        r = residual.contiguous()
+    if bias is not None and (bias.dtype != torch.float32 or tuple(bias.shape) != (Nw,) or not bias.is_contiguous()):
+        return None
+    triple = ops._ln_triple(name, ln, Nw, False)
+    if triple is None:
+        return None
+    lw, lb, leps = triple
+    lib = _lib.load()
+    ws = torch.empty(int(lib.univs_cross_attention_workspace(L, S, N, H)), dtype=torch.float32, device=q.device)
+    plan = ctypes.c_int(0)
+    if not ops._call(name, lib.univs_cross_attention_partials_f32, q, ops._ptr(q), ops._ptr(k), ops._ptr(v), ops._opt(mask), ops._opt(flags),
+                     gen, L, S, N, H, 32, ldq, ldk, ldv, float(scale), ops._ptr(ws), ctypes.byref(plan)):
+        return None
+    y = torch.empty((L, N, Nw), dtype=torch.float32, device=q.device)
+    wp, winv = ops.presplit_weights(weight)
+    ok = ops._call(name, lib.univs_small_linear_merged_presplit_f32, q, ops._ptr(ws), ws.numel(), plan.value, L, N, H, ops._ptr(wp),
+                   ops._ptr(winv), ops._opt(bias), Nw, 0, ops._opt(r), ops._opt(lw), ops._opt(lb), leps, Nw, ops._ptr(y))
+    if not ok:
+        raise _lib.UnivsHipError(f"{name}: the out-projection refused the plan {plan.value} of L={L} N={N} H={H} after the partials ran")
+    return y
diff --git a/univs_amd/inference/video_entity.py b/univs_amd/inference/video_entity.py
--- a/univs_amd/inference/video_entity.py
+++ b/univs_amd/inference/video_entity.py
@@ -1,3 +1,4 @@
+import contextlib
 import math
 from typing import Tuple
 
@@ -177,7 +178,9 @@
     if not mine:
         return {}, None
     feats = model.backbone(x[mine] if mine != list(range(mine[0], mine[0] + len(mine))) else x[mine[0]:mine[0] + len(mine)])
-    mf, bfe, _enc, ms = model.sem_seg_head.pixel_decoder.forward_features(feats)
+    pd = model.sem_seg_head.pixel_decoder
+    with getattr(pd, "normed_optional", contextlib.nullcontext)():
+        mf, bfe, _enc, ms = pd.forward_features(feats)
     return {f: k for k, f in enumerate(mine)}, (mf, bfe, list(ms))
 
 
@@ -439,7 +442,8 @@
                     head = model.sem_seg_head
                     if (self.pixel_decoder_once_per_window and self.num_frames_window_test > T and stride < T
                             and hasattr(head, "pixel_decoder") and hasattr(head, "predictor")):
-                        mf, bfe, _enc, ms = head.pixel_decoder.forward_features(feats_window)
+                        with getattr(head.pixel_decoder, "normed_optional", contextlib.nullcontext)():
+                            mf, bfe, _enc, ms = head.pixel_decoder.forward_features(feats_window)
                         win_pd = (mf, bfe, list(ms))
                 o = i - win_start
                 if win_pd is not None:
diff --git a/univs_amd/layers.py b/univs_amd/layers.py
--- a/univs_amd/layers.py
+++ b/univs_amd/layers.py
@@ -45,14 +45,6 @@
 
     def convolve(self, x):
         y = None
-        if (SWITCHES.split_conv and x.is_cuda and self.kernel_size == (1, 1) and self.stride == (1, 1) and self.padding == (0, 0)
-                and self.dilation == (1, 1) and self.groups == 1):
-            from . import ops
-            y = ops.conv1x1(x, self.weight, self.bias)
-        return y if y is not None else F.conv2d(x, self.weight, self.bias, self.stride, self.padding, self.dilation, self.groups)
-
-    def forward(self, x):
-        y = None
         if (SWITCHES.split_conv and x.is_cuda and self.bias is None and self.kernel_size == (3, 3) and self.stride == (1, 1)
                 and self.padding == (1, 1) and self.dilation == (1, 1) and self.groups == 1):
             from . import ops
@@ -61,7 +53,10 @@
               and self.dilation == (1, 1) and self.groups == 1):
             from . import ops
             y = ops.conv1x1(x, self.weight, self.bias)
-        x = y if y is not None else F.conv2d(x, self.weight, self.bias, self.stride, self.padding, self.dilation, self.groups)
+        return y if y is not None else F.conv2d(x, self.weight, self.bias, self.stride, self.padding, self.dilation, self.groups)
+
+    def forward(self, x):
+        x = self.convolve(x)
         if isinstance(self.norm, nn.GroupNorm) and x.dtype == torch.float32:
             from . import ops
             relu = self.activation is F.relu
@@ -195,6 +190,12 @@
                     m3 = ops.pad4_mask(attn_mask)
                 if m3.dim() == 2:
                     m3 = m3.view(1, L, m3.shape[-1])
+            if SWITCHES.fold_attn_merge and _small(q, self.out_proj.weight, self.out_proj.bias):
+                from . import fused_ops
+                tail = dict(residual=residual, ln=(norm.weight, norm.bias, norm.eps)) if norm is not None else {}
+                y = fused_ops.attention_out_proj(q, k, v, m3, h, 1.0 / math.sqrt(d), self.out_proj.weight, self.out_proj.bias, **tail)
+                if y is not None:
+                    return (y if norm is not None or residual is None else residual + y), None
             out = ops.cross_attention(q, k, v, m3, h, 1.0 / math.sqrt(d))
             if out is not None:
                 return project(out), None
diff --git a/univs_amd/modeling/backbone/swin.py b/univs_amd/modeling/backbone/swin.py
--- a/univs_amd/modeling/backbone/swin.py
+++ b/univs_amd/modeling/backbone/swin.py
@@ -340,6 +340,9 @@
                 (x_out, H, W, x, Wh, Ww), x_normed = self.layers[i](x, Wh, Ww), None
             if i in self.out_indices:
                 x_out = x_normed if x_normed is not None else layer_norm(getattr(self, f"norm{i}"), x_out)
+                if SWITCHES.swin_channels_last and x_out.is_cuda and not torch.is_grad_enabled() and x_out.is_contiguous():
+                    outs[f"res{i + 2}"] = x_out.view(-1, H, W, self.num_features[i]).permute(0, 3, 1, 2)
+                    continue
                 outs[f"res{i + 2}"] = ops.transpose_last2(x_out).view(-1, self.num_features[i], H, W)
         return outs
 
diff --git a/univs_amd/modeling/meta_arch/mask_former_head.py b/univs_amd/modeling/meta_arch/mask_former_head.py
--- a/univs_amd/modeling/meta_arch/mask_former_head.py
+++ b/univs_amd/modeling/meta_arch/mask_former_head.py
@@ -75,8 +75,8 @@
             raise ValueError(f"pixel decoder {self.pixel_decoder_name} is outside the hot path (SURVEY.md section 2)")
         if targets is not None and hasattr(self.predictor, "prefetch_prompts"):
             self.predictor.prefetch_prompts(targets, next(iter(features.values())).shape[0])
-        mask_features, mask_features_bfe_conv, enc_features, multi_scale_features = \
-            self.pixel_decoder.forward_features(features)
+        with self.pixel_decoder.normed_optional():
+            mask_features, mask_features_bfe_conv, enc_features, multi_scale_features = self.pixel_decoder.forward_features(features)
         if self.transformer_in_feature != "multi_scale_pixel_decoder":
             raise ValueError("only TRANSFORMER_IN_FEATURE='multi_scale_pixel_decoder' is on the hot path")
         return self.predictor(multi_scale_features, mask_features, mask_features_bfe_conv, mask, targets)
diff --git a/univs_amd/modeling/pixel_decoder/msdeformattn.py b/univs_amd/modeling/pixel_decoder/msdeformattn.py
--- a/univs_amd/modeling/pixel_decoder/msdeformattn.py
+++ b/univs_amd/modeling/pixel_decoder/msdeformattn.py
@@ -1,3 +1,4 @@
+import contextlib
 from typing import Callable, Dict, List, Optional, Union
 
 import numpy as np
@@ -5,7 +6,7 @@
 import torch.nn.functional as F
 from torch import nn
 
-from ... import ops
+from ... import fused_ops, ops
 from ...layers import Conv2d, get_activation_fn, get_norm, layer_norm, linear, linear_act
 from ...registry import SEM_SEG_HEADS_REGISTRY, ShapeSpec, configurable
 from ..position_encoding import PositionEmbeddingSine
@@ -326,15 +327,38 @@
             self._pe_cache[key] = p
         return p
 
+    @contextlib.contextmanager
+    def normed_optional(self):
+        old = self.__dict__.get("_normed_optional", False)
+        self.__dict__["_normed_optional"] = True
+        try:
+            yield self
+        finally:
+            self.__dict__["_normed_optional"] = old
+
     def forward_features(self, features):
+        want_normed = not self.__dict__.get("_normed_optional", False)
         with torch.autocast(device_type=next(iter(features.values())).device.type, enabled=False):
             if SWITCHES.graphs and not self.training and all(f.is_cuda for f in features.values()):
                 g = self.__dict__.get("_graphed")
                 if g is None:
                     from ...graphs import GraphedCallable
                     g = self.__dict__["_graphed"] = GraphedCallable(self._forward_features)
-                return g({k: features[k] for k in self.in_features})
-            return self._forward_features(features)
+                return g({k: features[k] for k in self.in_features}, bool(want_normed))
+            return self._forward_features(features, want_normed)
+
+    @staticmethod
+    def _conv1x1_in_place(conv, x):
+        if not x.is_cuda or x.is_contiguous() or not x.is_contiguous(memory_format=torch.channels_last):
+            return None, x
+        y = None
+        if SWITCHES.split_conv and x.dtype == torch.float32 and not ops.needs_grad(x, conv.weight, conv.bias):
+            y = fused_ops.conv1x1_fused(x, conv.weight, conv.bias)
+        if y is None:
+            T, C, H, W = x.shape
+            tokens = x.permute(0, 2, 3, 1).reshape(T, H * W, C)
+            x = ops.transpose_last2(tokens).view(T, C, H, W) if not ops.needs_grad(x) else x.contiguous()
+        return y, x
 
     def _input_proj(self, idx, x):
         conv, gn = self.input_proj[idx][0], self.input_proj[idx][1]
@@ -345,13 +369,15 @@
             return ops.group_norm(y, gn.num_groups, gn.weight, gn.bias, gn.eps)
         return self.input_proj[idx](x)
 
-    def _forward_features(self, features):
+    def _forward_features(self, features, want_normed=True):
         srcs, pos, affines = [], [], []
         for idx, f in enumerate(self.transformer_in_features[::-1]):
             x = features[f].float()
             conv, gn = self.input_proj[idx][0], self.input_proj[idx][1]
+            raw, x = self._conv1x1_in_place(conv, x)
             if x.is_cuda and not torch.is_grad_enabled() and not ops.needs_grad(x, conv.weight):
-                raw = ops.conv1x1(x, conv.weight, conv.bias) if SWITCHES.split_conv else None
+                if raw is None:
+                    raw = ops.conv1x1(x, conv.weight, conv.bias) if SWITCHES.split_conv else None
                 raw = conv(x) if raw is None else raw
                 srcs.append(raw)
                 affines.append(ops.group_norm_affine(raw, gn.num_groups, gn.weight, gn.bias, gn.eps))
@@ -370,13 +396,15 @@
             out = [ops.transpose_last2(z).view(bs, -1, spatial_shapes[i][0], spatial_shapes[i][1]) for i, z in enumerate(y)]
         else:
             out = [z.transpose(1, 2).reshape(bs, -1, spatial_shapes[i][0], spatial_shapes[i][1]) for i, z in enumerate(y)]
+        normed, folded = None, None
         for idx, f in enumerate(self.in_features[:self.num_fpn_levels][::-1]):
             x = features[f].float()
             lat = self.lateral_convs[idx]
             y_ = None
+            raw_in_place, x = self._conv1x1_in_place(lat, x)
             if (x.is_cuda and isinstance(lat.norm, nn.GroupNorm) and lat.activation is None and not torch.is_grad_enabled()
                     and x.shape[-2] == 2 * out[-1].shape[-2] and x.shape[-1] == 2 * out[-1].shape[-1]):
-                raw = lat.convolve(x)
+                raw = raw_in_place if raw_in_place is not None else lat.convolve(x)
                 y_ = ops.upsample2x_add(out[-1], raw, ops.group_norm_affine(raw, lat.norm.num_groups, lat.norm.weight, lat.norm.bias,
                                                                           lat.norm.eps))
                 if y_ is None:
@@ -385,6 +413,20 @@
             if y_ is None:
                 cur_fpn = lat(x)
                 y_ = ops.bilinear_resample(out[-1], cur_fpn.shape[-2:], addend=cur_fpn)
-            out.append(self.output_convs[idx](y_))
+            oc = self.output_convs[idx]
+            if (idx + 1 == self.num_fpn_levels and not want_normed and SWITCHES.fold_fpn_norm and SWITCHES.split_conv and y_.is_cuda
+                    and y_.dtype == torch.float32 and len(out) >= self.maskformer_num_feature_levels
+                    and isinstance(oc.norm, nn.GroupNorm) and oc.activation is F.relu and not torch.is_grad_enabled()
+                    and self.mask_features.norm is None and self.mask_features.activation is None):
+                raw = oc.convolve(y_)
+                affine = ops.group_norm_affine(raw, oc.norm.num_groups, oc.norm.weight, oc.norm.bias, oc.norm.eps)
+                folded = fused_ops.conv1x1_fused(raw, self.mask_features.weight, self.mask_features.bias, affine)
+                if folded is None:
+                    normed = ops.group_norm(raw, oc.norm.num_groups, oc.norm.weight, oc.norm.bias, oc.norm.eps, relu=True)
+                out.append(normed)
+                continue
+            out.append(oc(y_))
         multi_scale_features = out[:self.maskformer_num_feature_levels]
+        if folded is not None:
+            return folded, None, out[0], multi_scale_features
         return self.mask_features(out[-1]), out[-1], out[0], multi_scale_features
diff --git a/univs_amd/ops.py b/univs_amd/ops.py
--- a/univs_amd/ops.py
+++ b/univs_amd/ops.py
@@ -801,8 +801,7 @@
     return padded
 
 
-def cross_attention(q, k, v, mask, num_heads, scale):
-    _inference_only("cross_attention", q, k, v)
+def _cross_attention_args(q, k, v, mask, num_heads):
     if not (q.is_cuda and q.dtype == torch.float32 and k.dtype == torch.float32 and v.dtype == torch.float32):
         return None
     L, N, E = q.shape
@@ -831,9 +830,18 @@
             ld = E
         lds_.append((t, ld))
     (q, ldq), (k, ldk), (v, ldv) = lds_
+    return q, k, v, mask, flags, gen, L, S, N, H, ldq, ldk, ldv
+
+
+def cross_attention(q, k, v, mask, num_heads, scale):
+    _inference_only("cross_attention", q, k, v)
+    args = _cross_attention_args(q, k, v, mask, num_heads)
+    if args is None:
+        return None
+    q, k, v, mask, flags, gen, L, S, N, H, ldq, ldk, ldv = args
     lib = _lib.load()
     ws = torch.empty(int(lib.univs_cross_attention_workspace(L, S, N, H)), dtype=torch.float32, device=q.device)
-    out = torch.empty((L, N, E), dtype=torch.float32, device=q.device)
+    out = torch.empty((L, N, H * 32), dtype=torch.float32, device=q.device)
     ok = _call("cross_attention", lib.univs_cross_attention_flagged_f32, q, _ptr(q), _ptr(k), _ptr(v), _opt(mask), _opt(flags), gen,
                L, S, N, H, 32, ldq, ldk, ldv, float(scale), _ptr(ws), _ptr(out))
     return out if ok else None
diff --git a/univs_amd/switches.py b/univs_amd/switches.py
--- a/univs_amd/switches.py
+++ b/univs_amd/switches.py
@@ -30,6 +30,9 @@
     resident_presplit: bool = True
     sampler: str = "auto"
     graphs: bool = False
+    fold_fpn_norm: bool = True
+    fold_attn_merge: bool = False
+    swin_channels_last: bool = True
 
 
 SWITCHES = Switches(
@@ -40,7 +43,8 @@
     presplit_kmin=int(os.environ.get("UNIVS_PRESPLIT_KMIN", "768")), fused_mlp=_flag("UNIVS_FUSED_MLP", True),
     fused_cross_attention=_flag("UNIVS_FUSED_XATTN", True), fused_norm1=_flag("UNIVS_FUSED_NORM1", True), small_linear=_flag("UNIVS_SMALL_LINEAR", True),
     resident_presplit=_flag("UNIVS_RESIDENT_PRESPLIT", True), small_mlp_chain=_flag("UNIVS_SMALL_MLP_CHAIN", True), fused_proca=_flag("UNIVS_FUSED_PROCA", True),
-    fused_sampler=_flag("UNIVS_FUSED_SAMPLER", True), small_mlp_norm=_flag("UNIVS_SMALL_MLP_NORM", True))
+    fused_sampler=_flag("UNIVS_FUSED_SAMPLER", True), small_mlp_norm=_flag("UNIVS_SMALL_MLP_NORM", True),
+    fold_fpn_norm=_flag("UNIVS_FOLD_FPN_NORM", True), fold_attn_merge=_flag("UNIVS_FOLD_ATTN_MERGE", False), swin_channels_last=_flag("UNIVS_SWIN_CHANNELS_LAST", True))
 if SWITCHES.sampler not in ("auto", "reference", "device"):
     raise ValueError(f"UNIVS_SAMPLER={SWITCHES.sampler!r} (expected 'auto', 'reference' or 'device')")
 
```

Result: faster. 370.5 frames/s, median of 6 (+1.7%).
